# Kizuna42/office-person-detection-vit

Measured on AMD Instinct MI355X. Metric: frames/sec (Phase-2 DETR detect) at 800x1333 batch 8, higher is better.
Workload: dtype f16

## Files before the change

### office_person_detection_vit_amd/_capi.py

```python

from __future__ import annotations

import ctypes as C
import os
from typing import Optional

_HERE = os.path.dirname(os.path.abspath(__file__))
LIB_PATH = os.path.join(_HERE, "libopd_hip.so")
TEST_LIB_PATH = os.path.join(_HERE, "libopd_hip_test.so")

OPD_PIXELS_U8_BGR_HWC = 0
OPD_PIXELS_F32_NCHW = 1
OPD_MEM_HOST = 0
OPD_MEM_DEVICE = 1
OPD_MEM_HOST_PIXELS_DEVICE_OUT = 2
OPD_FLAG_NO_GRAPH = 1
OPD_FLAG_MULTI_STREAM = 2
OPD_REID_MODEL_CLIP = 0
OPD_REID_MODEL_OSNET = 1
OPD_FLAG_BF16 = 4
OPD_COMM_ID_BYTES = 128
OPD_OK, OPD_EINVAL, OPD_EIO, OPD_ESCHEMA, OPD_EHIP, OPD_ENOMEM, OPD_ESTATE = 0, -1, -2, -3, -4, -5, -6


# ... 39 lines not shown
    "opd_detr_forward_ragged": (C.c_int, [C.c_void_p, C.c_void_p, C.c_int, C.c_int, C.c_int, C.c_int, C.c_int, C.c_void_p,
                                          C.c_void_p, C.c_void_p, C.c_void_p]),
    "opd_detr_forward_resized": (C.c_int, [C.c_void_p, C.c_void_p] + [C.c_int] * 6 + [C.c_void_p] * 3),
    "opd_detr_resize_u8": (C.c_int, [C.c_void_p, C.c_void_p] + [C.c_int] * 5 + [C.c_void_p]),
    "opd_detr_detect_resized": (C.c_int, [C.c_void_p, C.c_void_p] + [C.c_int] * 6 + [C.c_float, C.POINTER(OpdDet), C.POINTER(C.c_int32)]),
    "opd_detr_detect_frames": (C.c_int, [C.c_void_p, C.POINTER(C.c_void_p)] + [C.c_int] * 6 + [C.c_float, C.POINTER(OpdDet), C.POINTER(C.c_int32)]),
    "opd_detr_detect_frames_features": (C.c_int, [C.c_void_p, C.POINTER(C.c_void_p)] + [C.c_int] * 5 + [C.c_float, C.c_int, C.POINTER(OpdDet), C.POINTER(C.c_int32),
                                                   C.POINTER(C.c_float)]),
    "opd_detr_postprocess": (C.c_int, [C.c_void_p, C.c_float, C.c_void_p, C.POINTER(OpdDet), C.POINTER(C.c_int32)]),
    "opd_detr_detect": (C.c_int, [C.c_void_p, C.c_void_p, C.c_int, C.c_int, C.c_int, C.c_int, C.c_int, C.c_float,
                                  C.c_void_p, C.POINTER(OpdDet), C.POINTER(C.c_int32)]),
    "opd_detr_detect_ragged": (C.c_int, [C.c_void_p, C.c_void_p, C.c_int, C.c_int, C.c_int, C.c_int, C.c_int, C.c_void_p,
                                         C.c_float, C.c_void_p, C.POINTER(OpdDet), C.POINTER(C.c_int32)]),
    "opd_detr_detect_async": (C.c_int, [C.c_void_p, C.c_void_p, C.c_int, C.c_int, C.c_int, C.c_int, C.c_int, C.c_float, C.c_void_p,
                                        C.POINTER(OpdDet), C.POINTER(C.c_int32), C.POINTER(C.c_int)]),
    "opd_detr_wait": (C.c_int, [C.c_void_p, C.c_int]),
    "opd_person_nms": (C.c_int, [C.POINTER(OpdDet), C.c_int, C.c_int, C.c_float]),
    "opd_person_nms_batch": (C.c_int, [C.POINTER(OpdDet), C.POINTER(C.c_int32), C.c_int, C.c_int, C.c_int, C.c_float]),
    "opd_host_alloc": (C.c_int, [C.c_size_t, C.POINTER(C.c_void_p)]),
    "opd_host_free": (None, [C.c_void_p]),
    "opd_similarity_matrix": (C.c_int, [C.c_int, C.c_void_p, C.c_void_p, C.c_void_p, C.c_int, C.c_void_p, C.c_void_p, C.c_void_p, C.c_int,
                                        C.c_int, C.c_double, C.c_double, C.c_int, C.c_void_p]),
    "opd_detr_roi_features": (C.c_int, [C.c_void_p, C.c_int, C.c_void_p, C.c_int, C.c_int, C.c_int, C.c_void_p]),
    "opd_detr_attention_map": (C.c_int, [C.c_void_p, C.c_int, C.c_int, C.c_void_p, C.c_int, C.c_void_p, C.c_int]),
    "opd_detr_set_profiling": (C.c_int, [C.c_void_p, C.c_int]),
    "opd_detr_stage_times": (C.c_int, [C.c_void_p, C.POINTER(C.c_float)]),
    "opd_detr_kernel_times": (C.c_int, [C.c_void_p, C.POINTER(C.c_float), C.POINTER(C.c_int32), C.POINTER(C.c_double)]),
    "opd_detr_kernel_table": (C.c_int, [C.c_void_p, C.c_void_p, C.c_int, C.POINTER(C.c_int)]),
    "opd_comm_available": (C.c_int, []),
    "opd_comm_unique_id": (C.c_int, [C.c_void_p]),
    "opd_comm_create": (C.c_int, [C.c_void_p, C.c_int, C.c_int, C.c_void_p, C.POINTER(C.c_void_p)]),
    "opd_comm_attach": (C.c_int, [C.c_void_p, C.c_void_p, C.POINTER(C.c_void_p)]),
    "opd_comm_destroy": (None, [C.c_void_p]),
    "opd_comm_info": (C.c_int, [C.c_void_p, C.POINTER(C.c_int), C.POINTER(C.c_int)]),
    "opd_comm_begin": (C.c_int, [C.c_void_p, C.c_int]),
    "opd_comm_detect": (C.c_int, [C.c_void_p, C.c_int, C.c_void_p, C.c_int, C.c_int, C.c_int, C.c_int, C.c_int, C.c_float, C.c_void_p]),
    "opd_comm_buffers": (C.c_int, [C.c_void_p, C.c_int, C.POINTER(C.c_void_p), C.POINTER(C.c_void_p)]),
    "opd_comm_exchange": (C.c_int, [C.c_void_p]),
    "opd_comm_wait": (C.c_int, [C.c_void_p, C.POINTER(OpdDet), C.POINTER(C.c_int32)]),
    "opd_reid_create": (C.c_int, [C.POINTER(OpdReidConfig), C.c_char_p, C.c_int, C.POINTER(C.c_void_p)]),
    "opd_reid_destroy": (None, [C.c_void_p]),
    "opd_reid_info": (C.c_int, [C.c_void_p, C.POINTER(OpdReidModelInfo)]),
    "opd_reid_extract": (C.c_int, [C.c_void_p, C.POINTER(C.c_void_p), C.c_void_p, C.c_int, C.c_int, C.c_void_p, C.c_void_p, C.c_int,
                                   C.c_void_p]),
    "opd_last_error": (C.c_char_p, []),
    "opd_version": (C.c_char_p, []),
}

TEST_API = {
    "opd_test_conv_gemm": (C.c_int, [C.c_void_p] * 6 + [C.c_int] * 15),
    "opd_test_gemm_splitk_ln": (C.c_int, [C.c_void_p] * 8 + [C.c_int] * 3),
    "opd_test_gemm_k256": (C.c_int, [C.c_void_p] * 5 + [C.c_int] * 5),
    "opd_test_gemm_ln": (C.c_int, [C.c_void_p] * 8 + [C.c_int] * 2),
    "opd_test_bench_gemm_ln": (C.c_int, [C.c_int] * 4 + [C.POINTER(C.c_float)]),
    "opd_test_gemm_ln_deep": (C.c_int, [C.c_void_p] * 7 + [C.c_int] + [C.c_void_p] * 3 + [C.c_int] * 3),
    "opd_test_set_heads2": (C.c_int, [C.c_int]),
    "opd_test_enc_ffn": (C.c_int, [C.c_void_p] * 9 + [C.c_int] + [C.c_void_p] * 3 + [C.c_int] * 3 + [C.c_void_p] * 2 + [C.c_int] * 2 + [C.c_void_p] * 5 + [C.c_int]),
    "opd_test_bench_enc_ffn": (C.c_int, [C.c_int] * 6 + [C.POINTER(C.c_float)]),
    "opd_test_bench_conv": (C.c_int, [C.c_int] * 11 + [C.POINTER(C.c_float)]),
    "opd_test_trace_btail": (C.c_int, [C.c_int] * 6 + [C.POINTER(C.c_ulonglong), C.c_int, C.POINTER(C.c_int)]),
    "opd_test_trace_conv": (C.c_int, [C.c_int] * 10 + [C.POINTER(C.c_ulonglong), C.c_int, C.POINTER(C.c_int)]),
    "opd_test_btail": (C.c_int, [C.c_void_p] * 10 + [C.c_int] * 6),
    "opd_test_bench_btail": (C.c_int, [C.c_int] * 8 + [C.POINTER(C.c_float)]),
    "opd_test_btail_repeat": (C.c_int, [C.c_void_p] * 8 + [C.c_int] * 6 + [C.POINTER(C.c_int)]),
    "opd_test_attention": (C.c_int, [C.c_void_p] * 4 + [C.c_int] * 4 + [C.c_float]),
    "opd_test_layernorm": (C.c_int, [C.c_void_p] * 5 + [C.c_int]),
    "opd_test_maxpool": (C.c_int, [C.c_void_p] * 2 + [C.c_int] * 6),
    "opd_test_preprocess_u8": (C.c_int, [C.c_void_p] * 2 + [C.c_int] * 5 + [C.c_void_p]),
    "opd_test_attention_masked": (C.c_int, [C.c_void_p] * 4 + [C.c_int] * 4 + [C.c_float, C.c_void_p, C.c_int]),
    "opd_test_stem2": (C.c_int, [C.c_void_p] * 4 + [C.c_int] * 5),
    "opd_test_stem_pool": (C.c_int, [C.c_void_p] * 4 + [C.c_int] * 7),
    "opd_test_set_fuse_stem_pool": (C.c_int, [C.c_void_p, C.c_int]),
    "opd_test_set_pos_shadow": (C.c_int, [C.c_void_p, C.c_int]),
    "opd_test_stem_pool_u8": (C.c_int, [C.c_void_p] * 6 + [C.c_int] * 3),
    "opd_test_set_fuse_btail": (C.c_int, [C.c_void_p, C.c_int]),
    "opd_test_set_fuse_gemm_ln": (C.c_int, [C.c_void_p, C.c_int]),
    "opd_test_f32_to_f16": (C.c_uint16, [C.c_float]),
    "opd_test_f16_to_f32": (C.c_float, [C.c_uint16]),
    "opd_test_normalise_key": (C.c_int, [C.c_char_p, C.c_char_p, C.c_int]),
    "opd_test_inspect_checkpoint": (C.c_int, [C.c_char_p, C.POINTER(C.c_int32)]),
    "opd_test_resize_coeffs": (C.c_int, [C.c_int, C.c_int, C.c_void_p, C.c_void_p, C.c_int]),
    "opd_test_valid_prefix": (C.c_int, [C.c_int] * 3),
    "opd_test_trunk_plan": (C.c_int, [C.c_void_p] + [C.c_int] * 6 + [C.c_void_p, C.c_int, C.c_void_p]),
    "opd_test_sine_pos_embed": (C.c_int, [C.c_int] * 5 + [C.c_void_p]),
    "opd_test_conv_dual": (C.c_int, [C.c_void_p] * 6 + [C.c_int] * 13),
    "opd_test_btail_sc": (C.c_int, [C.c_void_p] * 11 + [C.c_int] * 3),
    "opd_test_btail_chain": (C.c_int, [C.c_void_p] * 13 + [C.c_int] * 4),
    "opd_test_bench_attention": (C.c_int, [C.c_void_p] * 3 + [C.c_int] * 6 + [C.c_float, C.c_int, C.POINTER(C.c_float)]),
    "opd_test_trace_attention": (C.c_int, [C.c_void_p] * 3 + [C.c_int] * 6 + [C.c_float, C.c_void_p, C.c_int, C.POINTER(C.c_int)]),
    "opd_test_heads": (C.c_int, [C.c_void_p] * 13 + [C.c_int] * 2),
    "opd_test_postprocess": (C.c_int, [C.c_void_p] * 3 + [C.c_int] * 3 + [C.c_float, C.c_void_p, C.c_void_p]),
    "opd_test_roi_features": (C.c_int, [C.c_void_p] * 2 + [C.c_int] * 3 + [C.c_void_p]),
    "opd_test_set_conv_flags": (C.c_int, [C.c_int]),
    "opd_test_set_gemm_ln_kloop": (C.c_int, [C.c_int]),
    "opd_test_set_graph_guard": (C.c_int, [C.c_int]),
    "opd_test_set_alloc_poison": (C.c_int, [C.c_int]),
    "opd_test_check_redzones": (C.c_int, [C.c_void_p]),
    "opd_test_set_taps": (C.c_int, [C.c_void_p, C.c_int]),
    "opd_test_read_taps": (C.c_int, [C.c_void_p, C.c_void_p, C.c_int, C.c_char_p, C.c_int]),
    "opd_test_round_f16_diffused": (C.c_int, [C.c_void_p, C.c_int, C.c_int, C.c_int]),
    "opd_test_dec_qkv": (C.c_int, [C.c_void_p, C.c_void_p, C.c_int] + [C.c_void_p] * 5 + [C.c_int] * 2 + [C.c_void_p] * 4),
    "opd_test_dec_self": (C.c_int, [C.c_void_p] * 10 + [C.c_int, C.c_int, C.c_float, C.c_void_p]),
    "opd_test_attention_split": (C.c_int, [C.c_void_p] * 3 + [C.c_int] * 4 + [C.c_float, C.c_int, C.c_void_p, C.c_int, C.c_void_p, C.c_void_p]),
    "opd_test_dec_cross_out": (C.c_int, [C.c_void_p, C.c_void_p, C.c_int, C.c_void_p, C.c_int] + [C.c_void_p] * 4 + [C.c_int, C.c_void_p]),
    "opd_test_dec_ffn": (C.c_int, [C.c_void_p] * 4 + [C.c_int, C.c_int, C.c_void_p]),
    "opd_test_bench_dec": (C.c_int, [C.c_int] * 6 + [C.POINTER(C.c_float)]),
    "opd_test_heads_fused": (C.c_int, [C.c_void_p, C.c_void_p, C.c_int] + [C.c_void_p] * 13 + [C.c_int, C.c_int, C.c_void_p, C.c_void_p]),
    "opd_test_set_fused_dec": (C.c_int, [C.c_void_p, C.c_int]),
    "opd_test_set_elem_bf16": (C.c_int, [C.c_int]),
    "opd_test_trace_dec_self": (C.c_int, [C.c_int, C.c_int, C.c_void_p]),
    "opd_test_reid_geometry": (C.c_int, [C.c_void_p, C.c_int, C.c_int, C.c_int, C.c_void_p]),
    "opd_test_reid_coeffs": (C.c_int, [C.c_int] * 4 + [C.c_void_p, C.c_void_p, C.c_int]),
    "opd_test_reid_lut": (C.c_int, [C.c_void_p]),
    "opd_test_reid_pixels_host": (C.c_int, [C.c_void_p, C.c_int, C.c_int, C.c_void_p] + [C.c_int] * 3 + [C.c_void_p]),
    "opd_test_reid_pixels": (C.c_int, [C.c_void_p, C.POINTER(C.c_void_p), C.c_void_p, C.c_int, C.c_int, C.c_void_p, C.c_void_p, C.c_int,
                                       C.c_void_p]),
    "opd_test_reid_attention": (C.c_int, [C.c_void_p, C.c_void_p] + [C.c_int] * 3),
    "opd_test_reid_layernorm": (C.c_int, [C.c_void_p] * 5 + [C.c_int] * 3),
    "opd_test_reid_gemm": (C.c_int, [C.c_int, C.c_void_p, C.c_void_p, C.c_void_p, C.c_int, C.c_void_p] + [C.c_int] * 3),
    "opd_test_reid_l2norm": (C.c_int, [C.c_void_p] + [C.c_int] * 2),
    "opd_test_osnet_lut": (C.c_int, [C.c_void_p]),
    "opd_test_osnet_geometry": (C.c_int, [C.c_void_p, C.c_int, C.c_int, C.c_int, C.c_void_p]),
    "opd_test_osnet_pixels_host": (C.c_int, [C.c_void_p, C.c_int, C.c_int, C.c_void_p, C.c_int, C.c_void_p]),
    "opd_test_osnet_stem": (C.c_int, [C.c_void_p] * 4 + [C.c_int] * 2),
    "opd_test_osnet_gemm": (C.c_int, [C.c_int, C.c_void_p, C.c_int, C.c_int, C.c_void_p, C.c_int, C.c_int, C.c_void_p, C.c_void_p, C.c_void_p,
                                      C.c_int, C.c_void_p] + [C.c_int] * 6),
    "opd_test_osnet_dwconv": (C.c_int, [C.c_void_p] * 4 + [C.c_int] * 7),
    "opd_test_osnet_gate": (C.c_int, [C.c_void_p] * 7 + [C.c_int] * 4),
    "opd_test_osnet_avgpool2": (C.c_int, [C.c_void_p] * 2 + [C.c_int] * 4),
    "opd_test_osnet_head": (C.c_int, [C.c_void_p] * 4 + [C.c_int] * 3),
    "opd_test_reid_kernel_table": (C.c_int, [C.c_void_p, C.POINTER(C.c_void_p), C.c_void_p, C.c_int, C.c_void_p, C.c_void_p, C.c_int, C.c_int,
                                             C.POINTER(OpdKernelStat), C.c_int, C.POINTER(C.c_int)]),
}

_lib: Optional[C.CDLL] = None
_lib_has_hooks = False


def load_library(test_hooks: bool = False) -> C.CDLL:
    global _lib, _lib_has_hooks
    test_hooks = test_hooks or os.environ.get("OPD_TEST_HOOKS") == "1"
    if _lib is not None:
        if test_hooks and not _lib_has_hooks:
            raise RuntimeError("the product library is already loaded in this process; load the test build first "
                               "(_capi.load_library(test_hooks=True) or OPD_TEST_HOOKS=1)")
        return _lib
    path = TEST_LIB_PATH if test_hooks else LIB_PATH
    if not os.path.exists(path):
        raise RuntimeError(
            f"HIP extension not built: {path} is missing (run `python -c 'import __graft_entry__ as g; g.build()'`). "
            "This package has no CPU fallback.")
    lib = C.CDLL(path)
    for table in (API, TEST_API) if test_hooks else (API,):
        for name, (res, args) in table.items():
            fn = getattr(lib, name)
            fn.restype = res
            fn.argtypes = args
    _lib, _lib_has_hooks = lib, test_hooks
    return lib


def last_error() -> str:
    return load_library().opd_last_error().decode("utf-8", "replace")


def check(rc: int, what: str) -> None:
# ... 3 lines not shown
```

### office_person_detection_vit_amd/csrc/build.py

```python

from __future__ import annotations

import os
import subprocess
import sys

HERE = os.path.dirname(os.path.abspath(__file__))
PKG = os.path.dirname(HERE)
SOURCES = ["kernels_gemm.hip", "kernels_w8.hip", "kernels_btail.hip", "kernels_btail3.hip", "kernels_rowln.hip", "kernels_attn.hip", "kernels_misc.hip", "kernels_dec.hip", "kernels_reid.hip", "kernels_osnet.hip", "opd_loader.cpp", "opd_host.cpp", "opd_model.cpp", "opd_comm.cpp", "opd_dispatch.cpp", "opd_reid.cpp", "opd_osnet.cpp", "opd_test_api.cpp", "opd_reid_test_api.cpp", "opd_osnet_test_api.cpp"]
TEST_ONLY = {"opd_test_api.cpp", "opd_reid_test_api.cpp", "opd_osnet_test_api.cpp"}
ELEM_SOURCES = ["kernels_gemm.hip", "kernels_w8.hip", "kernels_btail.hip", "kernels_btail3.hip", "kernels_rowln.hip", "kernels_attn.hip", "kernels_misc.hip"]
HEADERS = ["opd_kernels.h", "opd_elem.h", "opd_loader.h", "opd_host.h", "opd_model.h", "opd_reid.h", "opd_osnet.h", os.path.join("..", "..", "include", "opd_detr.h")]
COMMON_FLAGS = ["-O3", "-fPIC", "-std=c++17", "--offload-arch=gfx950", "-Wall", "-Wno-unused-function", "-fvisibility=hidden"]
EXTRA_FLAGS = {"kernels_attn.hip": ["-mllvm", "-amdgpu-mfma-vgpr-form"]}
BF16_FLAGS = ["-DOPD_ELEM_BF16=1"]


def hipcc_path() -> str:
    return os.environ.get("HIPCC", "/opt/rocm/bin/hipcc")


LIB = os.path.join(PKG, "libopd_hip.so")
TEST_LIB = os.path.join(PKG, "libopd_hip_test.so")


def _stale(target: str, deps) -> bool:
    if not os.path.exists(target):
        return True
    t = os.path.getmtime(target)
    return any(os.path.getmtime(d) >= t for d in deps)


def build(verbose: bool = False, force: bool = False) -> str:
    hipcc = hipcc_path()
    objdir = os.path.join(HERE, "build")
    os.makedirs(objdir, exist_ok=True)
    hdrs = [os.path.join(HERE, h) for h in HEADERS]
    objs = []
    common, extra = COMMON_FLAGS, EXTRA_FLAGS
    jobs = []
    for src in SOURCES:
        sp = os.path.join(HERE, src)
        obj = os.path.join(objdir, os.path.splitext(src)[0] + ".o")
        objs.append(obj)
        if force or _stale(obj, [sp] + hdrs):
            jobs.append([hipcc] + common + extra.get(src, []) + (["-x", "hip"] if src.endswith(".cpp") else []) + ["-c", sp, "-o", obj])
        if src in ELEM_SOURCES:
            obj16 = os.path.join(objdir, os.path.splitext(src)[0] + "_bf16.o")
            objs.append(obj16)
            if force or _stale(obj16, [sp] + hdrs):
                jobs.append([hipcc] + common + extra.get(src, []) + BF16_FLAGS + ["-c", sp, "-o", obj16])

    def compile_one(cmd):
        if verbose:
            print(" ".join(cmd), flush=True)
        subprocess.run(cmd, check=True)

    if jobs:
        from concurrent.futures import ThreadPoolExecutor
        cores = int(os.environ.get("MAX_JOBS") or 0) or len(os.sched_getaffinity(0))
        with ThreadPoolExecutor(max_workers=max(1, min(len(jobs), cores))) as pool:
            list(pool.map(compile_one, jobs))
    test_objs = {os.path.join(objdir, os.path.splitext(s)[0] + ".o") for s in TEST_ONLY}
    for lib, members in ((LIB, [o for o in objs if o not in test_objs]), (TEST_LIB, objs)):
        if force or _stale(lib, members):
            cmd = [hipcc, "-shared", "-fPIC", "--offload-arch=gfx950", "-o", lib] + members + ["-ldl"]
            if verbose:
                print(" ".join(cmd), flush=True)
            subprocess.run(cmd, check=True)
    return LIB


if __name__ == "__main__":
    print(build(verbose=True, force="--force" in sys.argv))
```

### office_person_detection_vit_amd/csrc/kernels_btail.hip

```cpp
#include <hip/hip_runtime.h>
#include "opd_kernels.h"
#include "opd_elem.h"

typedef elem_t half8 __attribute__((ext_vector_type(8)));
typedef float float4v __attribute__((ext_vector_type(4)));
typedef unsigned int uint2v __attribute__((ext_vector_type(2)));
typedef unsigned int uint4v __attribute__((ext_vector_type(4)));

namespace {

constexpr int ROW_BYTES = 128;
constexpr int NW = 4;

__device__ __forceinline__ int swz(int row, int chunk) { return row * ROW_BYTES + ((chunk ^ (row & 7)) << 4); }

__device__ __forceinline__ int xcd_logical_block(int bid, int nblocks) {
    const int q = nblocks >> 3, r = nblocks & 7;
    const int x = bid & 7, k = bid >> 3;
    return (x < r ? x * (q + 1) : r * (q + 1) + (x - r) * q) + k;
}

__device__ __forceinline__ int own_row(const int rho) { return (rho & ~31) | (((rho >> 2) & 3) << 3) | (((rho >> 4) & 1) << 2) | (rho & 3); }
__device__ __forceinline__ int own_ch(const int nt, const int g) { return (nt >> 1) * 32 + g * 8 + (nt & 1) * 4; }

// ... 420 lines not shown
            }
        if constexpr (C3 > 0) {
            const unsigned char* W3s = W2s + W2C_BYTES;
#pragma unroll
            for (int kk = 0; kk < 2; ++kk) {
#pragma unroll
                for (int nt = 0; nt < NT3; ++nt) {
                    const half8 wf = *reinterpret_cast<const half8*>(W3s + swz(nt * 16 + li, kk * 4 + g));
#pragma unroll
                    for (int mt = 0; mt < 2; ++mt) accz[nt][mt] = OPD_MFMA_16x16x32(wf, yf[kk][mt], accz[nt][mt]);
                }
            }
        }
        if (j + 1 < NCH) {
            if (res_dma && j + 2 < NCH) wait_vmcnt<4>();
            else wait_vmcnt<0>();
            __builtin_amdgcn_s_barrier();
        }
#pragma unroll
        for (int q = 0; q < 2; ++q)
#pragma unroll
            for (int mt = 0; mt < 2; ++mt)
                if (y_ok[mt] && !(p.dbg & 2)) *reinterpret_cast<half8*>(p.y + pr_row[mt] + j * 64 + q * 32) = yf[q][mt];
        stamp(4 + j);
    }

    if constexpr (C3 > 0) {
#pragma unroll
        for (int q = 0; q < NT3 / 2; ++q)
#pragma unroll
            for (int mt = 0; mt < 2; ++mt) {
                float4v v0 = accz[2 * q][mt], v1 = accz[2 * q + 1][mt];
#pragma unroll
                for (int r = 0; r < 4; ++r) {
                    v0[r] = v0[r] > 0.f ? v0[r] : 0.f;
                    v1[r] = v1[r] > 0.f ? v1[r] : 0.f;
                }
                if (pr_ok[mt] && !(p.dbg & 2))
                    *reinterpret_cast<uint4*>(p.z + (size_t)(wm0 + mt * 16 + li) * C3 + q * 32 + g * 8) =
                        make_uint4(pack2h(v0[0], v0[1]), pack2h(v0[2], v0[3]), pack2h(v1[0], v1[1]), pack2h(v1[2], v1[3]));
            }
    }
    if constexpr (TRACE) {
        stamp(4 + NCH);
        asm volatile("s_waitcnt vmcnt(0)" ::: "memory");
        stamp(5 + NCH);
        asm volatile("s_memrealtime %0\n\ts_waitcnt lgkmcnt(0)" : "=s"(tstamp[15])::"memory");
        if (threadIdx.x == 0 && p.trace) {
#pragma unroll
            for (int i = 0; i < 16; ++i) p.trace[(size_t)blockIdx.x * 16 + i] = tstamp[i];
        }
    }
#endif
}

template <int C1, int C3, bool RDMA, bool SC = false, bool TRACE = false, int RC = 0>
hipError_t launch_btail_t(const BtailParams& p, hipStream_t stream) {
    constexpr int BM = 32 * NW;
    constexpr int MAIN = (BM + C1) * ROW_BYTES, CHUNK = 64 * C1 * 2 + C3 * ROW_BYTES + (SC ? 64 * ROW_BYTES : 0) + (RC ? 2 * 64 * ROW_BYTES : 0);
    constexpr int LDS = 2 * (MAIN > CHUNK ? MAIN : CHUNK) + (RDMA ? 2 * NW * 4096 : 0);
    static_assert(LDS <= 160 * 1024, "LDS per workgroup");
    OPD_SET_MAX_LDS_ONCE((btail_kernel<C1, C3, RDMA, SC, TRACE, RC>), LDS);
    OPD_LAUNCH((btail_kernel<C1, C3, RDMA, SC, TRACE, RC>), dim3((p.M + BM - 1) / BM), dim3(64 * NW), LDS, stream, p);
    static const char* const kname = opd_kernel_name("btail_kernel<%d, %d, %s, %s, %s, %d>", C1, C3, OPD_BOOLSTR(RDMA), OPD_BOOLSTR(SC), OPD_BOOLSTR(TRACE), RC);
    opd_last_kernel_name = kname;
    return hipGetLastError();
}

}

#ifndef OPD_ELEM_BF16
bool opd_btail_supported(int C1, int C3) {
    return (C1 == 64 && (C3 == 0 || C3 == 64 || C3 == 128)) || (C1 == 128 && (C3 == 0 || C3 == 128)) || opd_btail256_supported(C1, C3);
}
#endif

hipError_t OPD_SYM(opd_launch_btail)(const BtailParams& p_in, hipStream_t stream) {
    if (!opd_btail_supported(p_in.C1, p_in.C3) || p_in.OH <= 0 || p_in.OW <= 0) return hipErrorInvalidValue;
    BtailParams p = p_in;
    p.fd_ohw = opd_make_fastdiv((unsigned)p.OH * (unsigned)p.OW);
    p.fd_ow = opd_make_fastdiv((unsigned)p.OW);
    if ((size_t)p.B * p.H * p.W * p.C1 * 2 + (size_t)(p.W + 1) * p.C1 * 2 >= 0x7fffff00ull) return hipErrorInvalidValue;
    if ((size_t)p.M * p.C1 * 8 >= 0x7fffff00ull) return hipErrorInvalidValue;
    if (p.C1 == 256) return OPD_SYM(opd_launch_btail256)(p, stream);
    if (p.y_stride2 && (p.stride != 1 || p.C3 == 0)) return hipErrorInvalidValue;
    if (!p.y && !p.a1_out) return hipErrorInvalidValue;
    if (p.rc) {
        if (p.rc != 1 || p.C1 != 64 || p.C3 != 64 || p.stride != 1 || p.res || p.xs || !p.rc_a1 || !p.rc_xs || !p.rc_w2 || !p.rc_wsc || !p.rc_b ||
            p.trace || (size_t)p.M * 64 * 2 >= 0x7fffff00ull)
            return hipErrorInvalidValue;
        return launch_btail_t<64, 64, false, false, false, 1>(p, stream);
    }
    if (p.xs) {
        if (p.C1 != 64 || p.C3 != 64 || p.stride != 1 || !p.wsc || p.res || (size_t)p.M * 64 * 2 >= 0x7fffff00ull) return hipErrorInvalidValue;
        return launch_btail_t<64, 64, false, true>(p, stream);
    }
    if (p.trace) {
        if (p.C1 == 64 && p.C3 == 64 && (p.dbg & 16)) return launch_btail_t<64, 64, false, false, true>(p, stream);
        if (p.C1 == 64 && p.C3 == 64) return launch_btail_t<64, 64, true, false, true>(p, stream);
        if (p.C1 == 128 && p.C3 == 128) return launch_btail_t<128, 128, false, false, true>(p, stream);
        return hipErrorInvalidValue;
    }
    if (p.C1 == 64) {
        const bool rdma = !(p.dbg & 16);
        if (p.C3 == 0) return rdma ? launch_btail_t<64, 0, true>(p, stream) : launch_btail_t<64, 0, false>(p, stream);
        if (p.C3 == 64) return rdma ? launch_btail_t<64, 64, true>(p, stream) : launch_btail_t<64, 64, false>(p, stream);
        return rdma ? launch_btail_t<64, 128, true>(p, stream) : launch_btail_t<64, 128, false>(p, stream);
    }
    if (p.C3 == 0) return launch_btail_t<128, 0, false>(p, stream);
    return launch_btail_t<128, 128, false>(p, stream);
}

#ifndef OPD_ELEM_BF16
void opd_permute_k32(const f16_t* w, f16_t* out, int rows, int K) {
    for (int n = 0; n < rows; ++n)
        for (int b = 0; b < K; b += 32)
            for (int g = 0; g < 4; ++g)
                for (int e = 0; e < 4; ++e) {
                    out[(size_t)n * K + b + 8 * g + e] = w[(size_t)n * K + b + 4 * g + e];
                    out[(size_t)n * K + b + 8 * g + 4 + e] = w[(size_t)n * K + b + 16 + 4 * g + e];
                }
}
#endif
```

### office_person_detection_vit_amd/csrc/opd_kernels.h

```cpp
#pragma once
#include <hip/hip_runtime.h>
#include <stdint.h>
#include <vector>

typedef uint16_t f16_t;
enum { OPD_DT_F16 = 0, OPD_DT_BF16 = 1 };

#include <mutex>
#define OPD_SET_MAX_LDS_ONCE(kernel, bytes)                                                                                  \
    do {                                                                                                                     \
        static std::once_flag once_[16];                                                                                     \
        static hipError_t err_[16];                                                                                          \
        int dev_ = 0;                                                                                                        \
        if (hipGetDevice(&dev_) != hipSuccess || dev_ < 0 || dev_ >= 16) return hipErrorInvalidDevice;    \
        std::call_once(once_[dev_], [&] { err_[dev_] = hipFuncSetAttribute(reinterpret_cast<const void*>(kernel), hipFuncAttributeMaxDynamicSharedMemorySize, (bytes)); }); \
        if (err_[dev_] != hipSuccess) return err_[dev_];                                                                     \
    } while (0)

extern thread_local const char* opd_last_kernel_name;
extern thread_local int opd_dbg_skip_launch;
const char* opd_kernel_name(const char* fmt, ...);
#define OPD_LAUNCH(kernel, ...)                       \
    do {                                              \
        opd_last_kernel_name = #kernel;               \
// ... 7 lines not shown
        asm volatile("s_waitcnt vmcnt(0)" ::: "memory");         \
        __syncthreads();                                         \
    } while (0)
#else
#define OPD_DMA_BARRIER() __syncthreads()
#endif

struct FastDiv { unsigned mul, shift, one; };
inline FastDiv opd_make_fastdiv(unsigned d) {
    FastDiv f{0u, 0u, 1u};
    if (d <= 1u) return f;
    int s = 0;
    while ((1ull << s) < d) ++s;
    f.mul = (unsigned)(((1ull << (31 + s)) + d - 1) / d);
    f.shift = (unsigned)(s - 1);
    f.one = 0u;
    return f;
}

struct ConvGemmParams {
    const f16_t* x;
    const f16_t* w;
    const float* bias;
    const float* const* bias_ptrs;
    const f16_t* res16;
    const float* res32;
    void* out;
    f16_t* out16_aux;
    const void* zero16;
    int B, H, W, Cin, OH, OW, N, KH, KW, stride, pad;
    int M, K;
    int relu, bias_period, out_f32;
    int bias_pmod, bias_pcols;
    int stem;
    int dbg;
    int split_k;
    const f16_t* x2;
    int H2, W2, Cin2, stride2, K1;
    FastDiv fd_ohw, fd_ow, fd_period;
    const f16_t* x_alt;
    int alt_mod, alt_cols;
    unsigned tap_rep;
    FastDiv fd_tilesn, fd_ntiles;
    unsigned long long* trace;
    int force_mt;
    int wprefetch;
    int flat_staging;
    int dtype;
};
hipError_t opd_launch_conv_gemm(const ConvGemmParams& p, hipStream_t stream);
bool opd_conv_w8_supported(const ConvGemmParams& p);
hipError_t opd_launch_conv_w8(const ConvGemmParams& p, hipStream_t stream);
hipError_t opd_launch_stem_pool_u8(const uint8_t* frames, const int32_t* valid_hw, const f16_t* w, const float* bias, f16_t* out, int B, int H,
                                   int W, int OH, int OW, int PH, int PW, hipStream_t stream, int dtype = 0);
hipError_t opd_launch_stem_pool(const f16_t* x4p, const f16_t* w, const float* bias, f16_t* out, int B, int Hp, int Wp, int OH,
                                int OW, int PH, int PW, hipStream_t stream, int dtype = 0);
struct BtailParams {
    const f16_t* x1;
    const f16_t* w1;
    const float* b1;
    const f16_t* w2p;
    const float* b2;
    const f16_t* res;
    const f16_t* xs;
    const f16_t* wsc;
    f16_t* y;
    const f16_t* w3p;
    const float* b3;
    f16_t* z;
    int B, H, W, OH, OW, stride, M, C1, C3;
    int dbg;
    FastDiv fd_ohw, fd_ow;
    unsigned long long* trace;
    int rev;
    int dtype;
    f16_t* a1_out;
    const f16_t* rc_a1;
    const f16_t* rc_xs;
    const f16_t* rc_w2;
    const f16_t* rc_wsc;
    const float* rc_b;
    int rc;
    int y_stride2;
};
bool opd_btail_supported(int C1, int C3);
hipError_t opd_launch_btail(const BtailParams& p, hipStream_t stream);
void opd_permute_k32(const f16_t* w, f16_t* out, int rows, int K);
bool opd_btail256_supported(int C1, int C3);
hipError_t opd_launch_btail256(const BtailParams& p, hipStream_t stream);

struct GemmLnParams {
    const f16_t* x;
    const f16_t* w;
    const float* bias;
    const float* res32;
    const float* gamma;
    const float* beta;
    float* y32;
    f16_t* y16;
    int M, K;
    int kloop;
    int deep_k;
    const float* pos;
    const float* const* pos_ptrs;
    int pos_period;
    f16_t* yp16;
    int dtype;
};
hipError_t opd_launch_gemm_ln(const GemmLnParams& p, hipStream_t stream);
struct EncFfnParams {
    const f16_t* x;
    const unsigned char* wpack;
    const float* b2;
    const float* res32;
    const float* gamma;
    const float* beta;
    float* y32;
    f16_t* y16;
    f16_t* yp16;
    const float* pos;
    const float* const* pos_ptrs;
    int pos_period;
    int M, F;
    int dtype;
    int dbg;
    int wprefetch;
    const f16_t* attn;
    const float* bo;
    const float* gamma1;
    const float* beta1;
    int pack_front;
    int pack_tail;
    int tail, tail_pos;
    f16_t* tail_out;
    int tail_ld;
    int tail_col[16];
};
hipError_t opd_launch_enc_ffn(const EncFfnParams& p, hipStream_t stream);
size_t opd_encffn_pack_bytes(int F, int tail, int front);
void opd_encffn_pack(const uint16_t* w1, const float* b1, const uint16_t* w2, int F, const uint16_t* wt, const float* bt, int tail, const uint16_t* wo,
                     unsigned char* out);
struct GemmK256Params {
    const f16_t* x;
    const f16_t* w;
    const float* bias;
    f16_t* out16;
    float* out32;
    int M, N, ldx, ldw, slices, bias_period, relu;
    int dtype;
};
hipError_t opd_launch_gemm_k256(const GemmK256Params& p, hipStream_t stream);

hipError_t opd_launch_preprocess_u8(const uint8_t* frames, f16_t* out, int B, int H, int W, int Hp, int Wp, const int32_t* valid_hw,
                                    hipStream_t stream, int dtype = 0);
hipError_t opd_launch_preprocess_f32(const float* pv, f16_t* out, int B, int H, int W, int Hp, int Wp, const int32_t* valid_hw,
                                     hipStream_t stream, int dtype = 0);
void opd_resize_coeffs(int in_size, int out_size, std::vector<int32_t>* bounds, std::vector<int32_t>* coeffs, int* ksize_out);
hipError_t opd_launch_resize_u8(const uint8_t* in, uint8_t* out, int B, int h, int w, int oh, int ow, const int32_t* bounds_h,
                                const int32_t* coeff_h, int ksize_h, const int32_t* bounds_v, const int32_t* coeff_v, int ksize_v,
                                hipStream_t stream);
hipError_t opd_launch_maxpool(const f16_t* x, f16_t* out, int B, int H, int W, int C, int OH, int OW, hipStream_t stream, int dtype = 0);
hipError_t opd_launch_layernorm(const float* x, const float* gamma, const float* beta, float* y, f16_t* y16,
                                int rows, hipStream_t stream, int dtype = 0);
hipError_t opd_launch_reduce_ln(const float* partials, int nsplit, size_t slab_stride, const float* residual,
                                const float* gamma, const float* beta, float* y, f16_t* y16, int rows, hipStream_t stream, int dtype = 0);
hipError_t opd_launch_reduce_ln_pos(const float* partials, int nsplit, size_t slab_stride, const float* residual, const float* gamma,
                                    const float* beta, float* y, f16_t* y16, int rows, const float* pos, const float* const* pos_ptrs,
                                    int period, f16_t* yp16, hipStream_t stream, int dtype = 0);
hipError_t opd_launch_broadcast_rows(const float* c, float* y, f16_t* y16, int rows, hipStream_t stream, int dtype = 0);
hipError_t opd_launch_cast_f16(const float* x, f16_t* y, size_t n, hipStream_t stream, int dtype = 0);
hipError_t opd_launch_reduce_act16(const float* partials, int nsplit, size_t slab_stride, f16_t* out, size_t n, int relu, hipStream_t stream, int dtype = 0);
#define OPD_TAP_BLOCKS 64
// ... 35 lines not shown
hipError_t opd_launch_similarity_matrix(const float* f1, const float* b1, const uint8_t* has1, int n1, const float* f2, const float* b2,
                                        const uint8_t* has2, int n2, int D, double aw, double mw, int as_distance, float* out,
                                        hipStream_t stream);

void opd_split_f16_frag(const float* w, int N, int K, f16_t* out);
struct DecQkvParams {
    const float* h_in;
    const float* partials;
    int nsplit;
    const float* b2;
    const float *ln_g, *ln_b;
    float* h_out;
    const f16_t* w;
    const float* bias;
    f16_t* q16;
    f16_t* k16;
    f16_t* vT;
    int M, Q;
};
hipError_t opd_launch_dec_qkv(const DecQkvParams& p, hipStream_t stream);
struct DecSelfParams {
    const f16_t *q16, *k16, *vT;
    float* h;
    const f16_t* wo;
    const float *bo, *ln_g, *ln_b;
    const f16_t* wq;
    const float* rbq;
    f16_t* qc16;
    int qc_bf16;
    int B, Q;
    float scale;
    unsigned long long* trace;
};
hipError_t opd_launch_dec_self(const DecSelfParams& p, hipStream_t stream);
struct DecCrossOutParams {
    const float* part_o;
    const float* part_ml;
    int splits;
    const float* res;
    int res_period;
    float* h;
    const f16_t* wo;
    const float *bo, *ln_g, *ln_b;
    int M;
};
hipError_t opd_launch_dec_cross_out(const DecCrossOutParams& p, hipStream_t stream);
#define OPD_DEC_FFN_CHUNK 128
struct DecFfnParams {
    const float* h;
    const f16_t* w1;
    const float* b1;
    const f16_t* w2;
    float* partials;
    int M, F;
};
hipError_t opd_launch_dec_ffn(const DecFfnParams& p, hipStream_t stream);

struct AttnParams {
    const f16_t *q, *k, *v;
    f16_t* o;
    int B, heads, Lq, Lk;
    int ldq, ldk, ldv, ldo;
    float scale;
    const int32_t* key_valid;
    int key_row;
    unsigned long long* trace;
    int splits;
    float *part_o, *part_ml;
    int dtype;
};
hipError_t opd_launch_attention(const AttnParams& p, hipStream_t stream);

#define OPD_DECL_ELEM(name, ...)          \
    hipError_t name##_f16(__VA_ARGS__);   \
    hipError_t name##_bf16(__VA_ARGS__);
OPD_DECL_ELEM(opd_launch_conv_gemm, const ConvGemmParams& p, hipStream_t stream)
OPD_DECL_ELEM(opd_launch_conv_w8, const ConvGemmParams& p, hipStream_t stream)
OPD_DECL_ELEM(opd_launch_stem_pool_u8, const uint8_t* frames, const int32_t* valid_hw, const f16_t* w, const float* bias, f16_t* out, int B, int H, int W, int OH,
              int OW, int PH, int PW, hipStream_t stream)
OPD_DECL_ELEM(opd_launch_stem_pool, const f16_t* x4p, const f16_t* w, const float* bias, f16_t* out, int B, int Hp, int Wp, int OH, int OW, int PH, int PW,
              hipStream_t stream)
OPD_DECL_ELEM(opd_launch_btail, const BtailParams& p, hipStream_t stream)
OPD_DECL_ELEM(opd_launch_btail256, const BtailParams& p, hipStream_t stream)
OPD_DECL_ELEM(opd_launch_gemm_ln, const GemmLnParams& p, hipStream_t stream)
OPD_DECL_ELEM(opd_launch_enc_ffn, const EncFfnParams& p, hipStream_t stream)
OPD_DECL_ELEM(opd_launch_gemm_k256, const GemmK256Params& p, hipStream_t stream)
OPD_DECL_ELEM(opd_launch_attention, const AttnParams& p, hipStream_t stream)
OPD_DECL_ELEM(opd_launch_attention_map, const f16_t* q, int ldq, const f16_t* k, int ldk, const int32_t* sel, int nsel, int heads, int Lk, float scale,
              const int32_t* key_valid2, int key_row, void* stat, float* out, hipStream_t stream)
OPD_DECL_ELEM(opd_launch_preprocess_u8, const uint8_t* frames, f16_t* out, int B, int H, int W, int Hp, int Wp, const int32_t* valid_hw, hipStream_t stream)
OPD_DECL_ELEM(opd_launch_preprocess_f32, const float* pv, f16_t* out, int B, int H, int W, int Hp, int Wp, const int32_t* valid_hw, hipStream_t stream)
OPD_DECL_ELEM(opd_launch_maxpool, const f16_t* x, f16_t* out, int B, int H, int W, int C, int OH, int OW, hipStream_t stream)
OPD_DECL_ELEM(opd_launch_layernorm, const float* x, const float* gamma, const float* beta, float* y, f16_t* y16, int rows, hipStream_t stream)
OPD_DECL_ELEM(opd_launch_broadcast_rows, const float* c, float* y, f16_t* y16, int rows, hipStream_t stream)
OPD_DECL_ELEM(opd_launch_reduce_ln, const float* partials, int nsplit, size_t slab_stride, const float* residual, const float* gamma, const float* beta, float* y,
              f16_t* y16, int rows, hipStream_t stream)
OPD_DECL_ELEM(opd_launch_reduce_ln_pos, const float* partials, int nsplit, size_t slab_stride, const float* residual, const float* gamma, const float* beta,
              float* y, f16_t* y16, int rows, const float* pos, const float* const* pos_ptrs, int period, f16_t* yp16, hipStream_t stream)
OPD_DECL_ELEM(opd_launch_cast_f16, const float* x, f16_t* y, size_t n, hipStream_t stream)
OPD_DECL_ELEM(opd_launch_reduce_act16, const float* partials, int nsplit, size_t slab_stride, f16_t* out, size_t n, int relu, hipStream_t stream)
```

### office_person_detection_vit_amd/csrc/opd_model.cpp

```cpp
#include <new>
#include <stdexcept>

#include "opd_model.h"

using namespace opd;


namespace opd {

std::atomic<int> g_alloc_poison{-1};

static int upload_f32(opd_detr* m, float** dst, const std::vector<float>& v) {
    RCCHK(dalloc(m, dst, v.size(), true));
    HIPCHK(hipMemcpy(*dst, v.data(), v.size() * 4, hipMemcpyHostToDevice));
    return OPD_OK;
}
static int upload_f16(opd_detr* m, f16_t** dst, const std::vector<float>& v) {
    std::vector<f16_t> h(v.size());
    if (m->dtype == OPD_DT_BF16) for (size_t i = 0; i < v.size(); ++i) h[i] = f32_to_bf16(v[i]);
    else for (size_t i = 0; i < v.size(); ++i) h[i] = f32_to_f16(v[i]);
    RCCHK(dalloc(m, dst, h.size(), true));
    HIPCHK(hipMemcpy(*dst, h.data(), h.size() * 2, hipMemcpyHostToDevice));
    return OPD_OK;
}
// ... 587 lines not shown

static int run_small_gemm(opd_detr* m, const f16_t* x, const f16_t* w, const float* bias, int bias_period, int M, int N, int K,
                          f16_t* out16, bool relu) {
    GemmK256Params p{}; p.dtype = m->dtype;
    p.x = x; p.w = w; p.bias = bias; p.out16 = out16; p.M = M; p.N = N; p.ldx = K; p.ldw = K; p.slices = 1;
    p.bias_period = bias_period; p.relu = relu ? 1 : 0;
    RCCHK(timed_begin(m, CLS_GEMM, 2.0 * M * (double)N * K));
    HIPCHK(opd_launch_gemm_k256(p, m->stream));
    RCCHK(timed_end(m));
    RCCHK(tap(m, "gemm_k256", out16, (size_t)M * N * 2));
    return OPD_OK;
}
static int run_small_gemm_ln(opd_detr* m, const f16_t* x, const f16_t* w, const float* bias, int M, int K, const float* res32,
                             const LNp& ln, float* y32, f16_t* y16) {
    GemmK256Params p{}; p.dtype = m->dtype;
    p.x = x; p.w = w; p.bias = bias; p.out32 = m->d_slab; p.M = M; p.N = 256; p.ldx = K; p.ldw = K; p.slices = K / 256;
    RCCHK(timed_begin(m, CLS_GEMM, 2.0 * M * 256.0 * K));
    HIPCHK(opd_launch_gemm_k256(p, m->stream));
    RCCHK(timed_end(m));
    RCCHK(timed_begin(m, CLS_OTHER, 0.0));
    HIPCHK(opd_launch_reduce_ln(m->d_slab, p.slices, (size_t)M * 256, res32, ln.g, ln.b, y32, y16, M, m->stream, m->dtype));
    RCCHK(timed_end(m));
    RCCHK(tap(m, "small_gemm_ln", y32, (size_t)M * 256 * 4));
    return OPD_OK;
}

static int run_attn(opd_detr* m, const f16_t* q, int ldq, const f16_t* k, int ldk, const f16_t* v, int ldv, f16_t* o, int ldo,
                    int B, int Lq, int Lk, const int32_t* key_valid = nullptr, int key_row = 0) {
    AttnParams p{}; p.dtype = m->dtype;
    p.key_valid = key_valid; p.key_row = key_row;
    p.q = q; p.k = k; p.v = v; p.o = o; p.B = B; p.heads = m->arch.heads; p.Lq = Lq; p.Lk = Lk;
    p.ldq = ldq; p.ldk = ldk; p.ldv = ldv; p.ldo = ldo;
    p.scale = 1.0f / sqrtf((float)(m->arch.d_model / m->arch.heads));
    RCCHK(timed_begin(m, CLS_ATTN, 4.0 * B * (double)m->arch.heads * Lq * Lk * 32));
    HIPCHK(opd_launch_attention(p, m->stream));
    RCCHK(timed_end(m));
    if (ldo == m->arch.d_model) RCCHK(tap(m, "attention", o, (size_t)B * Lq * ldo * 2));
    return OPD_OK;
}

TrunkPlan plan_trunk(const Arch& a, const std::vector<Block>& blocks, const opd_config& cfg, const Switches& sw, int B, int H2, int W2, int num_cus,
                     bool taps, int profiling, bool has_stream2) {
    TrunkPlan plan;
    plan.steps.resize(blocks.size());
    plan.split = B;
    const bool multi = (cfg.flags & OPD_FLAG_MULTI_STREAM) != 0;
    int ch = H2, cw = W2, oh3 = 0, ow3 = 0;
    for (int s = 0, bi = 0; s < 4; ++s) {
        for (int l = 0; l < a.depths[s]; ++l, ++bi) {
            const Block& b = blocks[bi];
            const Block* nbk = bi + 1 < (int)blocks.size() ? &blocks[bi + 1] : nullptr;
            const int oh = (b.c1.stride == 2) ? down2(ch) : ch, ow = (b.c1.stride == 2) ? down2(cw) : cw;
            const int C1 = b.c1.Cin;
            const bool sc_in_tail = b.has_sc && sw.fuse_shortcut && sw.fuse_btail && block_has_bias2sc(b) && b.sc.KH == 1 && b.sc.stride == 1 &&
                                    b.sc.Cin == 64 && b.c1.Cin == 64 && b.c1.stride == 1 && b.c2.Cout == 256 && nbk && conv_has_kperm(nbk->c0) &&
                                    nbk->c0.Cin == 256 && nbk->c0.Cout == 64;
            bool tail = sw.fuse_btail && b.c1.KH == 3 && b.c1.Cout == C1 && b.c2.Cin == C1 && b.c2.Cout == 4 * C1 && conv_has_kperm(b.c2) &&
                        opd_btail_supported(C1, 0);
            if (sw.dual_over_tail && tail && b.has_sc && !sc_in_tail && block_has_w2sc(b)) tail = false;
            if (C1 == 256 && tail) {
                const long long tiles = ((long long)cfg.max_batch * oh * ow + 127) / 128;
                const bool pays = tiles * 10 >= (long long)num_cus * 6;
                if (sw.tail3 == 0 || (sw.tail3 == 1 && !pays && !multi)) tail = false;
            }
            const bool sc_in_expand = b.has_sc && sw.fuse_shortcut && block_has_w2sc(b) && !sc_in_tail && !tail;
            tail = tail && (size_t)B * ch * cw * C1 * 2 < 0x7ff00000ull;
            TrunkStep& t = plan.steps[bi];
            t.path = tail ? PATH_TAIL : sc_in_expand ? PATH_DUAL : PATH_CONVS;
            t.sc = !b.has_sc ? SC_NONE : (sc_in_tail && tail) ? SC_TAIL : sc_in_expand ? SC_EXPAND : SC_LAUNCH;
            t.res = (t.sc == SC_TAIL || t.sc == SC_EXPAND) ? RES_NONE : t.sc == SC_LAUNCH ? RES_SHORTCUT : RES_TRUNK;
            t.store = STORE_Y;
            t.C3 = 0;
            if (tail && nbk && conv_has_kperm(nbk->c0) && nbk->c0.Cin == 4 * C1 && opd_btail_supported(C1, nbk->c0.Cout)) t.C3 = nbk->c0.Cout;
            if (tail && sw.y_stride2 && t.C3 && b.c1.stride == 1 && l + 1 == a.depths[s] && nbk && nbk->has_sc && nbk->sc.stride == 2 && nbk->sc.KH == 1 &&
                nbk->c1.stride == 2 && !taps)
                t.store = STORE_Y_STRIDE2;
            if (l > 0 && sw.tail_rc && !taps) {
                TrunkStep& prev = plan.steps[bi - 1];
                if (prev.path == PATH_TAIL && prev.sc == SC_TAIL && prev.C3 == 64 && prev.store == STORE_Y && tail && C1 == 64 && t.C3 == 64 &&
                    t.res == RES_TRUNK) {
                    prev.store = STORE_A1;
                    t.res = RES_REBUILD;
                }
            }
            if (s == 2 && l == 0) { oh3 = oh; ow3 = ow; }
            ch = oh; cw = ow;
        }
    }
    const int s3 = a.depths[0] + a.depths[1], s4 = s3 + a.depths[2];
    bool fused3 = a.depths[2] > 2 && profiling != 1 && !taps && has_stream2 && sw.tail3_split && !multi && B >= 2;
    for (int bi = s3 + 1; bi < s4 && fused3; ++bi) fused3 = plan.steps[bi].path == PATH_TAIL;
    if (fused3) {
        auto tiles_of = [&](int frames) { return ((long long)frames * oh3 * ow3 + 127) / 128; };
        const long long total = tiles_of(B), cus = num_cus, last = total % cus;
        if (total > cus && last > 0 && last < cus / 2) {
            const long long whole = (total / cus) * cus;
            int bA = B - 1;
            while (bA > 1 && tiles_of(bA) > whole) --bA;
            if (tiles_of(bA) <= whole) plan.split = bA;
        }
    }
    int n = 0;
    auto rev = [&](const TrunkStep& t) { return t.path == PATH_TAIL && sw.tail_rev ? (n++ & 1) : 0; };
    for (int bi = 0; bi < s4; ++bi) plan.steps[bi].rev = rev(plan.steps[bi]);
    for (int bi = s3 + 1; bi < s4 && plan.split < B; ++bi) plan.steps[bi].rev_b = rev(plan.steps[bi]);
    for (int bi = s4; bi < (int)blocks.size(); ++bi) plan.steps[bi].rev = rev(plan.steps[bi]);
    return plan;
}

#define MARK(i)                                                   \
    do {                                                          \
        if (m->profiling) HIPCHK(hipEventRecord(m->ev[i], m->stream)); \
        opd_dbg_skip_launch = (m->sw.dbg_skip >> (i)) & 1;           \
    } while (0)

static bool is_ragged(const int32_t* valid_hw, int B, int H, int W) {
    if (!valid_hw) return false;
    for (int b = 0; b < B; ++b)
        if (valid_hw[2 * b] != H || valid_hw[2 * b + 1] != W) return true;
    return false;
}

static int enqueue_forward(opd_detr* m, const void* d_pixels, int pixel_format, int B, int H, int W, const int32_t* valid_hw = nullptr) {
    const Arch& a = m->arch;
    Dims d;
    compute_dims(B, H, W, &d);
    const int fh = d.sh[3], fw = d.sw[3];
    const bool ragged = is_ragged(valid_hw, B, H, W);
    Plan* plan = nullptr;
    const float* const* enc_bias_ptrs[16] = {};
    const float* const* kv_bias_ptrs = nullptr;
    const float* const* pos_ptrs = nullptr;
    const int32_t *d_valid = nullptr, *d_keyv = nullptr;
    if (!ragged) {
        RCCHK(get_plan(m, fh, fw, fh, fw, &plan));
    } else {
        if (a.enc_layers > 16) return fail(OPD_EINVAL, "ragged batches: at most 16 encoder layers");
        m->h_valid_hw.assign(valid_hw, valid_hw + 2 * B);
        m->h_key_valid.resize((size_t)2 * B);
        m->h_bias_ptrs.assign((size_t)(a.enc_layers + 2) * B, nullptr);
        for (int b = 0; b < B; ++b) {
            const int vh = valid_hw[2 * b], vw = valid_hw[2 * b + 1];
            if (vh < 1 || vw < 1 || vh > H || vw > W) return fail(OPD_EINVAL, "valid_hw outside the frame canvas");
            const int vfh = valid_prefix(vh, H, fh), vfw = valid_prefix(vw, W, fw);
            if (vfh < 1 || vfw < 1) return fail(OPD_EINVAL, "frame too small: no valid feature-map position");
            m->h_key_valid[2 * b] = vfh; m->h_key_valid[2 * b + 1] = vfw;
            Plan* pb = nullptr;
            RCCHK(get_plan(m, fh, fw, vfh, vfw, &pb));
            if (b == 0) plan = pb;
            for (int i = 0; i < a.enc_layers; ++i) m->h_bias_ptrs[(size_t)i * B + b] = pb->rb_enc[i];
            m->h_bias_ptrs[(size_t)a.enc_layers * B + b] = pb->rb_kv;
            m->h_bias_ptrs[(size_t)(a.enc_layers + 1) * B + b] = pb->d_pos;
        }
        HIPCHK(hipMemcpyAsync(m->d_valid_hw, m->h_valid_hw.data(), (size_t)2 * B * 4, hipMemcpyHostToDevice, m->stream));
        HIPCHK(hipMemcpyAsync(m->d_key_valid, m->h_key_valid.data(), (size_t)2 * B * 4, hipMemcpyHostToDevice, m->stream));
        HIPCHK(hipMemcpyAsync(m->d_bias_ptrs, m->h_bias_ptrs.data(), m->h_bias_ptrs.size() * sizeof(float*), hipMemcpyHostToDevice, m->stream));
        for (int i = 0; i < a.enc_layers; ++i) enc_bias_ptrs[i] = m->d_bias_ptrs + (size_t)i * B;
        kv_bias_ptrs = m->d_bias_ptrs + (size_t)a.enc_layers * B;
        pos_ptrs = m->d_bias_ptrs + (size_t)(a.enc_layers + 1) * B;
        d_valid = m->d_valid_hw;
        d_keyv = m->d_key_valid;
    }
    timed_reset(m);
    m->tap_next = 0;
    if (pixel_format == OPD_PIXELS_U8_BGR_HWC) RCCHK(tap(m, "pixels_u8", d_pixels, (size_t)B * H * W * 3));
    MARK(0);
    const int Hp = 2 * d.H1 + 6, Wp = 2 * d.W1 + 6;
    const bool prep_in_stem = m->sw.fuse_prep && m->sw.fuse_stem_pool && pixel_format == OPD_PIXELS_U8_BGR_HWC;
    if (!prep_in_stem) {
        RCCHK(timed_begin(m, CLS_OTHER, 0.0));
        if (pixel_format == OPD_PIXELS_U8_BGR_HWC)
            HIPCHK(opd_launch_preprocess_u8(reinterpret_cast<const uint8_t*>(d_pixels), m->d_x4, B, H, W, Hp, Wp, d_valid, m->stream, m->dtype));
        else
            HIPCHK(opd_launch_preprocess_f32(reinterpret_cast<const float*>(d_pixels), m->d_x4, B, H, W, Hp, Wp, d_valid, m->stream, m->dtype));
        RCCHK(timed_end(m));
    }
    if (prep_in_stem) {
        RCCHK(timed_begin(m, CLS_CONV, 2.0 * B * d.H1 * d.W1 * 64.0 * 147.0));
        HIPCHK(opd_launch_stem_pool_u8(reinterpret_cast<const uint8_t*>(d_pixels), d_valid, m->stem.w, m->stem.bias, m->d_pool, B, H, W, d.H1, d.W1,
                                       d.H2, d.W2, m->stream, m->dtype));
        RCCHK(timed_end(m));
        RCCHK(tap(m, "stem_pool_u8", m->d_pool, (size_t)B * d.H2 * d.W2 * 64 * 2));
    } else if (m->sw.fuse_stem_pool) {
        RCCHK(timed_begin(m, CLS_CONV, 2.0 * B * d.H1 * d.W1 * 64.0 * 147.0));
        HIPCHK(opd_launch_stem_pool(m->d_x4, m->stem.w, m->stem.bias, m->d_pool, B, Hp, Wp, d.H1, d.W1, d.H2, d.W2, m->stream, m->dtype));
        RCCHK(timed_end(m));
    } else {
        ConvGemmParams p{}; p.dtype = m->dtype;
        p.x = m->d_x4; p.w = m->stem.w; p.bias = m->stem.bias; p.out = m->d_stem; p.zero16 = m->zero_bias;
        p.B = B; p.H = Hp; p.W = Wp; p.Cin = 256; p.OH = d.H1; p.OW = d.W1; p.N = 64; p.KH = 1; p.KW = 1; p.stride = 2; p.pad = 0;
        p.M = B * d.H1 * d.W1; p.K = 256; p.relu = 1; p.stem = 2;
        RCCHK(timed_begin(m, CLS_CONV, 2.0 * p.M * 64.0 * 147.0));
        HIPCHK(opd_launch_conv_gemm(p, m->stream));
        RCCHK(timed_end(m));
        RCCHK(timed_begin(m, CLS_OTHER, 0.0));
        HIPCHK(opd_launch_maxpool(m->d_stem, m->d_pool, B, d.H1, d.W1, 64, d.H2, d.W2, m->stream, m->dtype));
        RCCHK(timed_end(m));
    }
    MARK(1);
    const TrunkPlan tp = plan_trunk(a, m->blocks, m->cfg, m->sw, B, d.H2, d.W2, m->num_cus, m->taps != 0, m->profiling, m->stream2 != nullptr);
    struct TrunkState { int cur_id; int ch, cw; int z_id; int prev_id; };
    auto run_blocks = [&](int s_begin, int s_end, int b0, int nb, TrunkState& st, int l_begin = 0, int l_end = 1 << 30) -> int {
        auto trunk = [&](int id, size_t per_frame) { return (id == 0 ? m->d_pool : id == 1 ? m->d_t0 : m->d_t1) + (size_t)b0 * per_frame; };
        auto mid = [&](int id, size_t per_frame) { return (id ? m->d_m1 : m->d_m0) + (size_t)b0 * per_frame; };
        for (int s = s_begin; s < s_end; ++s) {
            for (int l = l_begin; l < a.depths[s] && l < l_end; ++l) {
                const int bi = m->stage_first[s] + l;
                const Block& b = m->blocks[bi];
                const TrunkStep& t = tp.steps[bi];
                const int ch = st.ch, cw = st.cw;
                const int oh = (b.c1.stride == 2) ? down2(ch) : ch, ow = (b.c1.stride == 2) ? down2(cw) : cw;
                const int C1 = b.c1.Cin, C2 = b.c2.Cout, C3 = t.C3;
                const f16_t* cur = trunk(st.cur_id, (size_t)ch * cw * b.c0.Cin);
                const int out_id = st.cur_id == 1 ? 2 : 1;
                f16_t* out = trunk(out_id, (size_t)oh * ow * C2);
                f16_t* const scb = m->d_sc + (size_t)b0 * oh * ow * C2;
                if (t.sc == SC_LAUNCH) RCCHK(run_conv(m, b.sc, cur, nb, ch, cw, oh, ow, scb, false, nullptr));
                const f16_t* res = t.res == RES_TRUNK ? cur : t.res == RES_SHORTCUT ? scb : nullptr;
                int x1_id = st.z_id;
                const f16_t* x1 = nullptr;
                if (x1_id >= 0) {
                    x1 = mid(x1_id, (size_t)ch * cw * C1);
                } else {
                    x1_id = 0;
                    f16_t* c0out = mid(0, (size_t)ch * cw * b.c0.Cout);
                    RCCHK(run_conv(m, b.c0, cur, nb, ch, cw, ch, cw, c0out, true, nullptr, (l == 0 && s > 0) ? s - 1 : s));
                    x1 = c0out;
                }
                st.z_id = -1;
                if (t.path == PATH_TAIL) {
                    const Block* nbk = C3 ? &m->blocks[bi + 1] : nullptr;
                    BtailParams p{}; p.dtype = m->dtype;
                    p.x1 = x1; p.w1 = b.c1.w; p.b1 = b.c1.bias; p.w2p = C1 == 256 ? b.c2.wp : b.c2.w; p.b2 = b.c2.bias; p.res = res;
                    p.y = t.store == STORE_A1 ? nullptr : out;
                    if (t.sc == SC_TAIL) { p.xs = cur; p.wsc = b.sc.w; p.b2 = b.bias2sc; }
                    f16_t* z = mid(1 - x1_id, (size_t)oh * ow * C3);
                    if (C3) { p.w3p = C1 == 256 ? nbk->c0.wp : nbk->c0.w; p.b3 = nbk->c0.bias; p.z = z; }
                    f16_t* const a1_keep = m->d_sc + (size_t)b0 * oh * ow * C1;
                    if (t.store == STORE_A1) p.a1_out = a1_keep;
                    if (t.res == RES_REBUILD) {
                        const Block& pb = m->blocks[bi - 1];
                        p.rc = 1; p.rc_a1 = a1_keep; p.rc_xs = trunk(st.prev_id, (size_t)ch * cw * pb.c0.Cin); p.rc_w2 = pb.c2.w; p.rc_wsc = pb.sc.w; p.rc_b = pb.bias2sc;
                    }
                    p.y_stride2 = t.store == STORE_Y_STRIDE2;
                    p.B = nb; p.H = ch; p.W = cw; p.OH = oh; p.OW = ow; p.stride = b.c1.stride; p.M = nb * oh * ow; p.C1 = C1; p.C3 = C3;
                    p.rev = b0 ? t.rev_b : t.rev;
                    p.dbg = m->sw.dbg_btail;
                    RCCHK(timed_begin(m, CLS_CONV, 2.0 * p.M * ((double)C1 * 9 * C1 + 4.0 * C1 * C1 + 4.0 * C1 * C3 + (t.sc == SC_TAIL ? 64.0 * 256 : 0.0))));
                    HIPCHK(opd_launch_btail(p, m->stream));
                    RCCHK(timed_end(m));
                    if (p.y) RCCHK(tap(m, "btail_y", out, (size_t)p.M * 4 * C1 * 2));
                    if (C3) RCCHK(tap(m, "btail_z", z, (size_t)p.M * C3 * 2));
                    if (C3) st.z_id = 1 - x1_id;
                } else {
                    f16_t* a1 = mid(1 - x1_id, (size_t)oh * ow * C1);
                    RCCHK(run_conv(m, b.c1, x1, nb, ch, cw, oh, ow, a1, true, nullptr, s));
                    if (t.path == PATH_DUAL) {
                        ConvGemmParams p{}; p.dtype = m->dtype;
                        p.x = a1; p.w = b.w2sc; p.bias = b.bias2sc; p.out = out; p.zero16 = m->zero_bias;
                        p.B = nb; p.H = oh; p.W = ow; p.Cin = C1; p.OH = oh; p.OW = ow; p.N = C2; p.KH = 1; p.KW = 1; p.stride = 1; p.pad = 0;
                        p.M = nb * oh * ow; p.K1 = C1; p.K = C1 + b.sc.Cin; p.relu = 1;
                        p.x2 = cur; p.H2 = ch; p.W2 = cw; p.Cin2 = b.sc.Cin; p.stride2 = b.sc.stride; p.dbg = m->sw.dbg_gemm; p.wprefetch = m->sw.wprefetch & 1;
                        RCCHK(timed_begin(m, CLS_CONV, 2.0 * p.M * (double)C2 * p.K));
                        HIPCHK(opd_launch_conv_gemm(p, m->stream));
                        RCCHK(timed_end(m));
                        RCCHK(tap(m, "dual_expand", out, (size_t)p.M * C2 * 2));
                    } else {
                        RCCHK(run_conv(m, b.c2, a1, nb, oh, ow, oh, ow, out, true, res));
                    }
                }
                st.prev_id = st.cur_id; st.cur_id = out_id; st.ch = oh; st.cw = ow;
            }
            if (b0 + nb == B && l_end >= a.depths[s]) MARK(2 + s);
        }
        return OPD_OK;
    };
    TrunkState st{0, d.H2, d.W2, -1, -1};
    RCCHK(run_blocks(0, 2, 0, B, st));
    const int nbA = tp.split;
    RCCHK(run_blocks(2, 3, 0, B, st, 0, 1));
    if (nbA < B) {
        TrunkState ta = st, tb = st;
        HIPCHK(hipEventRecord(m->ev_fork, m->stream));
        HIPCHK(hipStreamWaitEvent(m->stream2, m->ev_fork, 0));
        hipStream_t main_stream = m->stream;
        const int rc_a = run_blocks(2, 3, 0, nbA, ta, 1);
        m->stream = m->stream2;
        const int rc_b = rc_a == OPD_OK ? run_blocks(2, 3, nbA, B - nbA, tb, 1) : OPD_OK;
        m->stream = main_stream;
        const hipError_t ej = hipEventRecord(m->ev_join, m->stream2);
        const hipError_t ew = ej == hipSuccess ? hipStreamWaitEvent(m->stream, m->ev_join, 0) : ej;
        RCCHK(rc_a);
        RCCHK(rc_b);
        HIPCHK(ew);
        MARK(4);
        st = ta;
    } else {
        RCCHK(run_blocks(2, 3, 0, B, st, 1));
    }
    RCCHK(run_blocks(3, 4, 0, B, st));
    const f16_t* cur = st.cur_id == 1 ? m->d_t0 : m->d_t1;
    const int ch = st.ch, cw = st.cw;
    const int hw = ch * cw, M = B * hw, D = a.d_model, F = a.ffn;
    const bool shadow = m->sw.pos_shadow && D == 256 && m->enc[0].bqkv && m->bkv_all;
    const PosShadow psh{plan->d_pos, pos_ptrs, hw, m->d_xp16};
    const PosShadow* ps = shadow ? &psh : nullptr;
    auto run_deep = [&](const f16_t* x, const Lin* lin, const f16_t* w, const float* bias, int K, const float* res32, const LNp* ln, int cls) -> int {
        GemmLnParams gp{}; gp.dtype = m->dtype;
        gp.x = x; gp.w = w; gp.bias = bias; gp.res32 = res32; gp.gamma = ln ? ln->g : nullptr; gp.beta = ln ? ln->b : nullptr;
        gp.y32 = m->d_x32; gp.y16 = m->d_x16; gp.M = M; gp.K = K; gp.deep_k = 1;
        if (ps) { gp.pos = ps->pos; gp.pos_ptrs = ps->pos_ptrs; gp.pos_period = ps->period; gp.yp16 = ps->yp16; }
        RCCHK(timed_begin(m, cls, 2.0 * M * (double)D * K));
        HIPCHK(opd_launch_gemm_ln(gp, m->stream));
        RCCHK(timed_end(m));
        RCCHK(tap(m, ln ? "fc2_ln_ring" : "input_proj_ring", m->d_x32, (size_t)M * D * 4));
        (void)lin;
        return OPD_OK;
    };
    const bool small_enc = m->sw.small_enc && (size_t)m->cfg.max_batch * m->stage_px[3] <= 1400;
    const int enc_splits = small_enc ? 8 : 4;
    const bool deep_ok = m->sw.deep_fc2 && D == 256 && !small_enc;
    if (deep_ok && m->proj.K % 64 == 0 && (size_t)M * m->proj.K * 2 < 0x7fffff00ull)
        RCCHK(run_deep(cur, nullptr, m->proj.w, m->proj.bias, m->proj.K, nullptr, nullptr, CLS_CONV));
    else
        RCCHK(run_gemm_splitk_ln(m, cur, m->proj.w, m->proj.bias, M, D, m->proj.K, (m->proj.K / 64) % enc_splits == 0 ? enc_splits : 4, nullptr, nullptr, m->d_x32, m->d_x16, CLS_CONV, ps));
    bool qkv_done = false, kv_done = false;
    const int Q = a.queries, Md = B * Q, NKV = a.dec_layers * 2 * D;
    for (int i = 0; i < a.enc_layers; ++i) {
        const EncLayer& L = m->enc[i];
        if (qkv_done) {
// ... 332 lines not shown
    }
    if (hw != m->h_orig_hw) {
        HIPCHK(hipStreamSynchronize(m->stream));
        m->h_orig_hw = hw;
        HIPCHK(hipMemcpyAsync(m->d_orig_hw, m->h_orig_hw.data(), m->h_orig_hw.size() * 4, hipMemcpyHostToDevice, m->stream));
    }
    PostParams pp{};
    pp.logits = m->d_logits; pp.boxes = m->d_boxes; pp.orig_hw = m->d_orig_hw;
    pp.records = dev_out ? dev_out : m->d_records;
    pp.counts = dev_counts ? dev_counts : m->d_counts;
    pp.B = B; pp.Q = m->arch.queries; pp.ncls = m->arch.ncls; pp.threshold = threshold;
    RCCHK(timed_begin(m, CLS_OTHER, 0.0));
    HIPCHK(opd_launch_postprocess(pp, m->stream));
    RCCHK(timed_end(m));
    MARK(8);
    return OPD_OK;
}

static int fetch_records(opd_detr* m, opd_det* out, int32_t* counts, int mem_kind, float* features = nullptr) {
    const int B = m->last_B, Q = m->arch.queries;
    if (!outputs_on_device(mem_kind)) {
        const size_t rec_bytes = (size_t)m->cfg.max_batch * Q * sizeof(opd_det);
        const size_t feat_off = reinterpret_cast<const char*>(m->d_feat_all) - reinterpret_cast<const char*>(m->d_records);
        const size_t feat_row = (size_t)Q * m->arch.d_model * 4;
        if (!m->sync_pinned) HIPCHK(hipHostMalloc(&m->sync_pinned, feat_off + (size_t)m->cfg.max_batch * feat_row, hipHostMallocDefault));
        HIPCHK(hipMemcpyAsync(m->sync_pinned, m->d_records, features ? feat_off + (size_t)B * feat_row : rec_bytes + (size_t)B * 4, hipMemcpyDeviceToHost, m->stream));
        HIPCHK(hipStreamSynchronize(m->stream));
        memcpy(out, m->sync_pinned, (size_t)B * Q * sizeof(opd_det));
        memcpy(counts, static_cast<char*>(m->sync_pinned) + rec_bytes, (size_t)B * 4);
        if (features) memcpy(features, static_cast<char*>(m->sync_pinned) + feat_off, (size_t)B * feat_row);
    }
    HIPCHK(hipStreamSynchronize(m->stream));
    if (m->profiling) {
        for (int i = 0; i < 8; ++i) {
            float ms = 0.f;
            hipEvent_t from = (i == 7 && m->profiling == 2 && m->graph_marks) ? m->ev[9] : m->ev[i];
            if (hipEventElapsedTime(&ms, from, m->ev[i + 1]) == hipSuccess) m->stage_ms[i] = ms;
            else (void)hipGetLastError();
        }
        if (m->profiling == 1) timed_collect(m);
    }
    return OPD_OK;
}

}

static hipError_t make_branch_stream(opd_detr* m) {
    hipError_t e = hipStreamCreateWithFlags(&m->stream2, hipStreamNonBlocking);
    if (e == hipSuccess) e = hipEventCreateWithFlags(&m->ev_fork, hipEventDisableTiming);
    if (e == hipSuccess) e = hipEventCreateWithFlags(&m->ev_join, hipEventDisableTiming);
    return e;
}
static void drop_streams(opd_detr* m) {
    if (m->ev_fork) (void)hipEventDestroy(m->ev_fork);
    if (m->ev_join) (void)hipEventDestroy(m->ev_join);
    if (m->stream2) (void)hipStreamDestroy(m->stream2);
    if (m->stream) (void)hipStreamDestroy(m->stream);
    m->ev_fork = m->ev_join = nullptr; m->stream2 = m->stream = nullptr;
}

static int create_impl(const opd_config* cfg, const char* weights_path, int device_ordinal, opd_detr** out);
static int clone_impl(const opd_detr* src, opd_detr** out);
template <typename F>
static int guarded(const char* what, F&& body) {
    try {
        return body();
    } catch (const std::bad_alloc&) {
        return fail(OPD_ENOMEM, std::string(what) + ": out of host memory");
    } catch (const std::out_of_range& e) {
        return fail(OPD_ESCHEMA, std::string(what) + ": weight file lacks a tensor the model needs (" + e.what() + ")");
    } catch (const std::exception& e) {
        return fail(OPD_EINVAL, std::string(what) + ": " + e.what());
    } catch (...) {
        return fail(OPD_EINVAL, std::string(what) + ": unknown C++ exception");
    }
}
static Switches read_switches(int flags) {
    Switches sw;
    auto env = [](const char* name, int* v) { if (const char* e = getenv(name)) *v = atoi(e); };
    env("OPD_DUAL_OVER_TAIL", &sw.dual_over_tail);
    env("OPD_TAIL_REV", &sw.tail_rev);
    env("OPD_TAIL3", &sw.tail3);
    env("OPD_TAIL_RC", &sw.tail_rc);
    sw.tail_rc = sw.tail_rc != 0;
    env("OPD_WPREFETCH", &sw.wprefetch);
    env("OPD_W8", &sw.w8);
    if (sw.w8 < 0) sw.w8 = (flags & OPD_FLAG_MULTI_STREAM) ? 1 : 0;
    env("OPD_SMALL_SPLITK", &sw.small_splitk);
    env("OPD_SMALL_ENC", &sw.small_enc);
    env("OPD_Y_STRIDE2", &sw.y_stride2);
    env("OPD_TAIL3_SPLIT", &sw.tail3_split);
    env("OPD_FUSE_PREP", &sw.fuse_prep);
    env("OPD_POS_SHADOW", &sw.pos_shadow);
    env("OPD_DEEP_FC2", &sw.deep_fc2);
    env("OPD_WROUND", &sw.wround);
    env("OPD_FUSED_DEC", &sw.fused_dec);
    env("OPD_FUSED_ENC_FFN", &sw.fused_enc_ffn);
    env("OPD_ENC_TAIL", &sw.enc_tail);
    env("OPD_ENC_FRONT", &sw.enc_front);
    env("OPD_HEADS2", &sw.heads2);
    env("OPD_DBG_DEC_LAYERS", &sw.dbg_dec_layers);
    env("OPD_DBG_BTAIL", &sw.dbg_btail);
    env("OPD_DBG_SKIP", &sw.dbg_skip);
    env("OPD_DBG_GEMM", &sw.dbg_gemm);
    return sw;
}

extern "C" {

const char* opd_version(void) { return "opd_hip 0.2 gfx950 (fp16 MFMA operands, fp32 accumulate; OPD_FLAG_BF16: bf16 operands)"; }

int opd_detr_create(const opd_config* cfg, const char* weights_path, int device_ordinal, opd_detr** out) {
    ApiScope api_scope;
    if (out) *out = nullptr;
    return guarded("opd_detr_create", [&] { return create_impl(cfg, weights_path, device_ordinal, out); });
}
int opd_detr_clone(const opd_detr* src, opd_detr** out) {
    ApiScope api_scope;
    if (out) *out = nullptr;
    return guarded("opd_detr_clone", [&] { return clone_impl(src, out); });
}
static int create_impl(const opd_config* cfg, const char* weights_path, int device_ordinal, opd_detr** out) {
    if (!cfg || !weights_path || !out) return fail(OPD_EINVAL, "opd_detr_create: null argument");
    if (cfg->struct_size != (int32_t)sizeof(opd_config)) return fail(OPD_EINVAL, "opd_config.struct_size mismatch");
    if (cfg->max_batch < 1 || cfg->max_height < 32 || cfg->max_width < 32) return fail(OPD_EINVAL, "opd_config maxima must be >= 1 x 32 x 32");
    *out = nullptr;
    StateDict sd;
    std::string err;
    int rc = load_safetensors(weights_path, &sd, &err);
    if (rc) return fail(rc, err);
    std::unique_ptr<opd_detr> m(new opd_detr());
    rc = infer_arch(sd, &m->arch, &err);
    if (rc) return fail(rc, err);
    m->cfg = *cfg;
    m->dtype = (cfg->flags & OPD_FLAG_BF16) ? OPD_DT_BF16 : OPD_DT_F16;
    m->sw = read_switches(cfg->flags);
    m->device = device_ordinal;
    int ndev = 0;
    if (hipGetDeviceCount(&ndev) != hipSuccess || ndev == 0)
        return fail(OPD_EHIP, "no HIP device visible (this library has no CPU fallback)");
    if (device_ordinal < 0 || device_ordinal >= ndev) return fail(OPD_EINVAL, "device_ordinal out of range");
    auto cleanup = [&](int code) {
        for (void* p : m->allocs) (void)hipFree(p);
        drop_streams(m.get());
        return code;
    };
    {
        hipError_t e = hipSetDevice(device_ordinal);
        if (e == hipSuccess) e = hipStreamCreateWithFlags(&m->stream, hipStreamNonBlocking);
        if (e == hipSuccess) e = make_branch_stream(m.get());
        if (e != hipSuccess) { drop_streams(m.get()); return fail(OPD_EHIP, std::string("device/stream setup failed: ") + hipGetErrorString(e)); }
        int cus = 0;
        if (hipDeviceGetAttribute(&cus, hipDeviceAttributeMultiprocessorCount, device_ordinal) == hipSuccess && cus > 0) m->num_cus = cus;
    }
    m->weights = std::make_shared<WeightSet>();
    m->weights->device = device_ordinal;
    if ((rc = build_weights(m.get(), sd))) return cleanup(rc);
    m->weights_sealed = true;
    if ((rc = build_workspace(m.get()))) return cleanup(rc);
    for (auto& e : m->ev)
        if (hipEventCreate(&e) != hipSuccess) return cleanup(fail(OPD_EHIP, "hipEventCreate failed"));
    *out = m.release();
    ++g_handle_epoch;
    return OPD_OK;
}

// ... 409 lines not shown
```

### office_person_detection_vit_amd/csrc/opd_model.h

```cpp
#pragma once
#include <math.h>
#include <stdlib.h>
#include <string.h>

#include <atomic>
#include <memory>
#include <mutex>
#include <shared_mutex>
#include <string>
#include <vector>

#include "../../include/opd_detr.h"
#include "opd_kernels.h"
#include "opd_loader.h"
#include "opd_host.h"

#define HIPCHK(expr)                                                                                           \
    do {                                                                                                       \
        hipError_t _e = (expr);                                                                                \
        if (_e != hipSuccess)                                                                                  \
            return opd::fail(OPD_EHIP, std::string(#expr) + " failed: " + hipGetErrorString(_e) + " (" + __FILE__ + \
                                           ":" + std::to_string(__LINE__) + ")");                              \
    } while (0)

// ... 7 lines not shown



struct Conv {
    f16_t* w = nullptr;
    f16_t* wp = nullptr;
    float* bias = nullptr;
    int Cin = 0, Cout = 0, KH = 1, KW = 1, stride = 1, pad = 0, K = 0;
    bool stem = false;
};
struct Lin {
    f16_t* w = nullptr;
    float* b = nullptr;
    int N = 0, K = 0;
};
struct LNp {
    float* g = nullptr;
    float* b = nullptr;
};
struct Block {
    Conv c0, c1, c2, sc;
    bool has_sc = false;
    float* bias2sc = nullptr;
    f16_t* w2sc = nullptr;
};
inline bool conv_has_kperm(const Conv& c) { return c.KH == 1 && c.KW == 1 && c.Cin % 32 == 0 && c.Cin <= 1024; }
inline bool block_has_bias2sc(const Block& b) { return b.has_sc && b.sc.Cout == b.c2.Cout; }
inline bool block_has_w2sc(const Block& b) {
    return block_has_bias2sc(b) && b.sc.KH == 1 && b.c2.KH == 1 && b.c2.Cout % 128 == 0 && b.c2.Cin >= 128;
}
struct EncLayer {
    f16_t* wqkv = nullptr;
    float* bqkv = nullptr;
    Lin o, fc1, fc2;
    LNp ln1, ln2;
    unsigned char* ffn_pack = nullptr;
    int tail = 0, tail_pos = 0, tail_ld = 0;
    int front = 0;
    int tail_col[16] = {};
};
struct DecLayer {
    f16_t* wqkv = nullptr;
    f16_t* wq_c = nullptr;
    Lin so, co, fc1, fc2;
    LNp ln1, ln2, ln3;
    float* rb_self = nullptr;
    float* rb_q = nullptr;
    f16_t *wqkv_f = nullptr, *so_f = nullptr, *wqc_f = nullptr, *co_f = nullptr, *fc1_f = nullptr, *fc2_f = nullptr;
};

struct Plan {
    int fh = 0, fw = 0;
    int vh = 0, vw = 0;
    std::vector<float*> rb_enc;
    float* rb_kv = nullptr;
    float* d_pos = nullptr;
};

struct Dims {
    int B, H, W, H1, W1, H2, W2;
    int sh[4], sw[4];
};

inline int down2(int n) { return (n - 1) / 2 + 1; }

struct Switches {
    int small_m_gemm = 1;
    int fuse_gemm_ln = 1;
    int deep_fc2 = 1;
    int fuse_dec0 = 1;
    int enc_front = 1;
    int enc_tail = 0;
    int fused_enc_ffn = 1;
    int fused_dec = 1;
    int dec_splits = 3;
    int heads2 = 1;
    int fuse_btail = 1;
    int fuse_shortcut = 1;
    int dual_over_tail = 1;
    int tail_rev = 1;
    int tail3 = 1;
    int tail3_split = 1;
    int tail_rc = 1;
    int y_stride2 = 1;
    int wprefetch = 3;
    int w8 = -1;
    int small_splitk = 1;
    int small_enc = 1;
    int fuse_stem_pool = 1;
    int fuse_prep = 1;
    int pos_shadow = 1;
    int wround = 1;
    int dbg_btail = 0, dbg_gemm = 0;
    int dbg_dec_layers = 1 << 20;
    int dbg_skip = 0;
};

enum TrunkPath { PATH_TAIL, PATH_CONVS, PATH_DUAL };
enum TrunkShortcut { SC_NONE, SC_TAIL, SC_EXPAND, SC_LAUNCH };
enum TrunkResidual { RES_NONE, RES_TRUNK, RES_SHORTCUT, RES_REBUILD };
enum TrunkStore { STORE_Y, STORE_A1, STORE_Y_STRIDE2 };
struct TrunkStep {
    int path, sc, res, store;
    int C3;
    int rev, rev_b;
};
struct TrunkPlan {
    std::vector<TrunkStep> steps;
    int split = 0;
};
TrunkPlan plan_trunk(const Arch& a, const std::vector<Block>& blocks, const opd_config& cfg, const Switches& sw, int B, int H2, int W2, int num_cus,
                     bool taps, int profiling, bool has_stream2);

}

using namespace opd;

struct RedZoned { void* base; size_t bytes; int poison; };
struct WeightSet {
    std::vector<void*> allocs;
    std::vector<RedZoned> zoned;
    int device = 0;
    std::mutex plan_mu;
    std::vector<std::unique_ptr<Plan>> plans;
    ~WeightSet() {
        (void)hipSetDevice(device);
        for (void* p : allocs) (void)hipFree(p);
    }
};

struct opd_detr {
    Arch arch;
    opd_config cfg{};
    Switches sw;
    int dtype = 0;
    int device = 0;
    hipStream_t stream = nullptr;
    hipStream_t stream2 = nullptr;
    hipEvent_t ev_fork = nullptr, ev_join = nullptr;
    std::vector<void*> allocs;
    std::vector<RedZoned> zoned;
    std::shared_ptr<WeightSet> weights;
    bool weights_sealed = false;
    int64_t weight_bytes = 0, workspace_bytes = 0;

    Conv stem;
    std::vector<Block> blocks;
    std::vector<int> stage_first;
    Conv proj;
    std::vector<EncLayer> enc;
    std::vector<DecLayer> dec;
    f16_t* wkv_all = nullptr;
    float* bkv_all = nullptr;
    float* dec0_h = nullptr;
    f16_t* qc0 = nullptr;
    LNp dec_ln;
    float *wc = nullptr, *bc = nullptr, *w1 = nullptr, *b1 = nullptr, *w2 = nullptr, *b2 = nullptr, *w3 = nullptr, *b3 = nullptr;
    f16_t *wc_f = nullptr, *w1_f = nullptr, *w2_f = nullptr;
    float* zero_bias = nullptr;

    std::vector<std::vector<float>> h_enc_cat_w, h_enc_cat_b;
    std::vector<float> h_kv_cat_w, h_kv_cat_b;

    uint8_t* d_u8 = nullptr;
    float* d_pv = nullptr;
    f16_t *d_x4 = nullptr, *d_stem = nullptr, *d_pool = nullptr, *d_t0 = nullptr, *d_t1 = nullptr, *d_m0 = nullptr,
          *d_m1 = nullptr, *d_sc = nullptr;
    float *d_x32 = nullptr, *d_y32 = nullptr, *d_slab = nullptr;
    f16_t* d_xp16 = nullptr;
    f16_t *d_x16 = nullptr, *d_qkv16 = nullptr, *d_attn16 = nullptr, *d_ffn16 = nullptr, *d_memkv16 = nullptr;
    float *d_h32 = nullptr, *d_yd32 = nullptr, *d_hs32 = nullptr;
    f16_t *d_h16 = nullptr, *d_qkvd16 = nullptr, *d_qd16 = nullptr, *d_attnd16 = nullptr, *d_ffnd16 = nullptr;
    f16_t *d_dq16 = nullptr, *d_dk16 = nullptr, *d_dvT = nullptr;
    float *d_part_o = nullptr, *d_part_ml = nullptr, *d_ffn_part = nullptr;
    float *d_logits = nullptr, *d_boxes = nullptr;
    opd_det* d_records = nullptr;
    int32_t *d_counts = nullptr, *d_orig_hw = nullptr;
    int32_t *d_valid_hw = nullptr, *d_key_valid = nullptr;
    const float** d_bias_ptrs = nullptr;
    std::vector<int32_t> h_valid_hw, h_key_valid;
    std::vector<const float*> h_bias_ptrs;
    hipEvent_t ev_async[4] = {};
    unsigned async_next = 0;
    bool async_pending[4] = {};
    struct AsyncHost { void* pinned = nullptr; opd_det* out = nullptr; int32_t* counts = nullptr; int B = 0; };
    AsyncHost async_host[4];
    void* sync_pinned = nullptr;
    float* d_feat_all = nullptr;
// ... 98 lines not shown
```

### office_person_detection_vit_amd/csrc/opd_test_api.cpp

```cpp
#include <string.h>

#include <string>
#include <cstring>
#include <vector>

#include "opd_model.h"

namespace {
int tfail(int code, const std::string& msg) {
    opd::g_err = msg;
    return code;
}
struct DevMem {
    std::vector<void*> ptrs;
    ~DevMem() {
        for (void* p : ptrs) (void)hipFree(p);
    }
    template <typename T>
    T* up(const T* host, size_t count) {
        void* d = nullptr;
        if (hipMalloc(&d, count * sizeof(T) + 16) != hipSuccess) return nullptr;
        ptrs.push_back(d);
        if (host && hipMemcpy(d, host, count * sizeof(T), hipMemcpyHostToDevice) != hipSuccess) return nullptr;
        return reinterpret_cast<T*>(d);
    }
};
#define TCHK(expr)                                                                                          \
    do {                                                                                                    \
        hipError_t _e = (expr);                                                                             \
        if (_e != hipSuccess) return tfail(OPD_EHIP, std::string(#expr) + ": " + hipGetErrorString(_e));    \
    } while (0)
}

#pragma GCC visibility push(default)
extern "C" {

static int g_conv_flags = 0, g_gemm_ln_kloop = 0, g_test_dtype = 0;
int opd_test_set_elem_bf16(int on) { g_test_dtype = on ? OPD_DT_BF16 : OPD_DT_F16; return OPD_OK; }
int opd_test_set_conv_flags(int flags) { g_conv_flags = flags; return OPD_OK; }
int opd_test_set_gemm_ln_kloop(int on) { g_gemm_ln_kloop = on ? 1 : 0; return OPD_OK; }
static void apply_conv_flags(ConvGemmParams& p, int flags) {
    p.force_mt = (flags >> 8) & 7;
    p.flat_staging = (flags >> 5) & 1;
}

int opd_test_conv_gemm(const uint16_t* x, const uint16_t* w, const float* bias, const uint16_t* res16, const float* res32,
                       void* out, int B, int H, int W, int Cin, int OH, int OW, int N, int KH, int KW, int stride, int pad,
                       int relu, int bias_period, int out_f32, int stem) {
    DevMem dm;
    const size_t M = (size_t)B * OH * OW;
    const int K = stem ? 256 : KH * KW * Cin;
    const size_t xin = (size_t)B * H * W * (stem ? 4 : Cin);
    ConvGemmParams p{}; p.dtype = g_test_dtype;
    p.x = dm.up(x, xin);
    p.w = dm.up(w, (size_t)N * K);
    p.bias = dm.up(bias, (size_t)N * (bias_period > 0 ? bias_period : 1));
    p.res16 = res16 ? dm.up(res16, M * N) : nullptr;
    p.res32 = res32 ? dm.up(res32, M * N) : nullptr;
    const size_t obytes = M * N * (out_f32 ? 4 : 2);
    p.out = dm.up<unsigned char>(nullptr, obytes);
    {
        const uint32_t zeros[8] = {0, 0, 0, 0, 0, 0, 0, 0};
        p.zero16 = dm.up(zeros, 8);
    }
    if (!p.zero16 || !p.x || !p.w || !p.bias || !p.out || (res16 && !p.res16) || (res32 && !p.res32)) return tfail(OPD_ENOMEM, "test alloc failed");
    p.B = B; p.H = H; p.W = W; p.Cin = Cin; p.OH = OH; p.OW = OW; p.N = N; p.KH = KH; p.KW = KW; p.stride = stride; p.pad = pad;
    p.M = (int)M; p.K = K; p.relu = relu; p.bias_period = bias_period; p.out_f32 = out_f32; p.stem = stem;
    apply_conv_flags(p, g_conv_flags);
    if (g_conv_flags & (1 << 12)) {
        if (!opd_conv_w8_supported(p)) return tfail(OPD_EINVAL, "conv_w8: shape outside the kernel's contract");
        TCHK(opd_launch_conv_w8(p, nullptr));
    } else {
        TCHK(opd_launch_conv_gemm(p, nullptr));
    }
    TCHK(hipDeviceSynchronize());
    TCHK(hipMemcpy(out, p.out, obytes, hipMemcpyDeviceToHost));
    return OPD_OK;
}

int opd_test_conv_dual(const uint16_t* x, const uint16_t* w1, const uint16_t* x2, const uint16_t* w2, const float* bias, uint16_t* out,
                       int B, int H, int W, int Cin, int KH, int stride, int pad, int N, int H2, int W2, int Cin2, int stride2, int relu) {
    DevMem dm;
    const int OH = (H + 2 * pad - KH) / stride + 1, OW = (W + 2 * pad - KH) / stride + 1;
    const size_t M = (size_t)B * OH * OW;
    const int K1 = KH * KH * Cin, K = K1 + Cin2;
    std::vector<uint16_t> wc((size_t)N * K);
    for (int n = 0; n < N; ++n) {
        memcpy(&wc[(size_t)n * K], w1 + (size_t)n * K1, (size_t)K1 * 2);
        memcpy(&wc[(size_t)n * K + K1], w2 + (size_t)n * Cin2, (size_t)Cin2 * 2);
    }
    ConvGemmParams p{}; p.dtype = g_test_dtype;
    p.x = dm.up(x, (size_t)B * H * W * Cin);
    p.x2 = dm.up(x2, (size_t)B * H2 * W2 * Cin2);
    p.w = dm.up(wc.data(), wc.size());
    p.bias = dm.up(bias, (size_t)N);
    p.out = dm.up<unsigned char>(nullptr, M * N * 2);
    const uint32_t zeros[8] = {0, 0, 0, 0, 0, 0, 0, 0};
    p.zero16 = dm.up(zeros, 8);
    if (!p.x || !p.x2 || !p.w || !p.bias || !p.out || !p.zero16) return tfail(OPD_ENOMEM, "test alloc failed");
    p.B = B; p.H = H; p.W = W; p.Cin = Cin; p.OH = OH; p.OW = OW; p.N = N; p.KH = KH; p.KW = KH; p.stride = stride; p.pad = pad;
    p.M = (int)M; p.K = K; p.K1 = K1; p.relu = relu; p.H2 = H2; p.W2 = W2; p.Cin2 = Cin2; p.stride2 = stride2;
    TCHK(opd_launch_conv_gemm(p, nullptr));
    TCHK(hipDeviceSynchronize());
    TCHK(hipMemcpy(out, p.out, M * N * 2, hipMemcpyDeviceToHost));
    return OPD_OK;
}

int opd_test_gemm_splitk_ln(const uint16_t* x, const uint16_t* w, const float* bias, const float* res32, const float* gamma,
                            const float* beta, float* y, uint16_t* y16, int M, int K, int splits) {
    DevMem dm;
    const int N = 256;
    ConvGemmParams p{}; p.dtype = g_test_dtype;
    p.x = dm.up(x, (size_t)M * K);
    p.w = dm.up(w, (size_t)N * K);
    p.bias = dm.up(bias, N);
    std::vector<float> zeros(N, 0.f);
    p.zero16 = dm.up(zeros.data(), N);
    float* slab = dm.up<float>(nullptr, (size_t)splits * M * N);
    const float* dres = res32 ? dm.up(res32, (size_t)M * N) : nullptr;
    const float* dg = gamma ? dm.up(gamma, N) : nullptr;
    const float* db = beta ? dm.up(beta, N) : nullptr;
// ... 218 lines not shown
    for (int i = 0; i < 2; ++i) TCHK(opd_launch_conv_gemm(p, nullptr));
    TCHK(hipEventRecord(a, nullptr));
    for (int i = 0; i < iters; ++i) TCHK(opd_launch_conv_gemm(p, nullptr));
    TCHK(hipEventRecord(b, nullptr));
    TCHK(hipEventSynchronize(b));
    float ms = 0.f;
    TCHK(hipEventElapsedTime(&ms, a, b));
    (void)hipEventDestroy(a); (void)hipEventDestroy(b);
    *us_out = ms * 1000.f / iters;
    return OPD_OK;
}

int opd_test_trace_conv(int B, int H, int W, int Cin, int N, int KH, int stride, int with_res, int split_k, int warm, unsigned long long* trace_out,
                        int max_wgs, int* wgs_out) {
    const int dbg = 0;
    DevMem dm;
    const int pad = KH / 2, OH = (H + 2 * pad - KH) / stride + 1, OW = (W + 2 * pad - KH) / stride + 1;
    const size_t M = (size_t)B * OH * OW, K = (size_t)KH * KH * Cin;
    ConvGemmParams p{}; p.dtype = g_test_dtype;
    uint16_t* x = dm.up<uint16_t>(nullptr, (size_t)B * H * W * Cin);
    uint16_t* w = dm.up<uint16_t>(nullptr, (size_t)N * K);
    float* bias = dm.up<float>(nullptr, N);
    uint16_t* res = with_res ? dm.up<uint16_t>(nullptr, M * N) : nullptr;
    uint16_t* out = dm.up<uint16_t>(nullptr, M * N * (split_k > 1 ? 2 * (size_t)split_k : 1));
    float* zero = dm.up<float>(nullptr, 4096);
    unsigned long long* tr = dm.up<unsigned long long>(nullptr, (size_t)max_wgs * 8);
    if (!x || !w || !bias || !out || !zero || !tr || (with_res && !res)) return tfail(OPD_ENOMEM, "trace alloc failed");
    TCHK(hipMemset(x, 0x2c, (size_t)B * H * W * Cin * 2));
    TCHK(hipMemset(w, 0x1c, (size_t)N * K * 2));
    TCHK(hipMemset(bias, 0, (size_t)N * 4));
    TCHK(hipMemset(zero, 0, 4096 * 4));
    TCHK(hipMemset(tr, 0, (size_t)max_wgs * 64));
    if (res) TCHK(hipMemset(res, 0x2c, M * N * 2));
    p.x = x; p.w = w; p.bias = bias; p.res16 = res; p.out = out; p.zero16 = zero;
    p.B = B; p.H = H; p.W = W; p.Cin = Cin; p.OH = OH; p.OW = OW; p.N = N; p.KH = KH; p.KW = KH; p.stride = stride; p.pad = pad;
    p.M = (int)M; p.K = (int)K; p.relu = 1; p.dbg = dbg;
    if (split_k > 1) { p.split_k = split_k; p.out_f32 = 1; p.relu = 0; }
    unsigned long long* tr3 = dm.up<unsigned long long>(nullptr, (size_t)3 * max_wgs * 8);
    if (!tr3) return tfail(OPD_ENOMEM, "trace alloc failed");
    TCHK(hipMemset(tr3, 0, (size_t)3 * max_wgs * 64));
    p.trace = tr;
    for (int i = 0; i < warm; ++i) TCHK(opd_launch_conv_gemm(p, nullptr));
    for (int i = 0; i < 3; ++i) {
        p.trace = tr3 + (size_t)i * max_wgs * 8;
        TCHK(opd_launch_conv_gemm(p, nullptr));
    }
    TCHK(hipDeviceSynchronize());
    TCHK(hipMemcpy(trace_out, tr3, (size_t)3 * max_wgs * 64, hipMemcpyDeviceToHost));
    const int bn = (N % 128 == 0) ? 128 : 64;
    (void)bn;
    *wgs_out = max_wgs;
    return OPD_OK;
}

int opd_test_btail(const uint16_t* x1, const uint16_t* w1, const float* b1, const uint16_t* w2, const float* b2,
                   const uint16_t* res, const uint16_t* w3, const float* b3, uint16_t* y, uint16_t* z, int B, int H, int W,
                   int C1, int C3, int stride) {
    if (!opd_btail_supported(C1, C3)) return tfail(OPD_EINVAL, "btail: unsupported (C1, C3)");
    DevMem dm;
    const int C2 = 4 * C1, OH = (H - 1) / stride + 1, OW = (W - 1) / stride + 1;
    const size_t M = (size_t)B * OH * OW;
    std::vector<uint16_t> w2p((size_t)C2 * C1), w3p((size_t)(C3 ? C3 : 1) * C2);
    if (C1 == 256) {
        opd_permute_k32(w2, w2p.data(), C2, C1);
        if (C3) opd_permute_k32(w3, w3p.data(), C3, C2);
    } else {
        w2p.assign(w2, w2 + (size_t)C2 * C1);
        if (C3) w3p.assign(w3, w3 + (size_t)C3 * C2);
    }
    BtailParams p{}; p.dtype = g_test_dtype;
    p.x1 = dm.up(x1, (size_t)B * H * W * C1);
    p.w1 = dm.up(w1, (size_t)C1 * 9 * C1);
    p.b1 = dm.up(b1, C1);
    p.w2p = dm.up(w2p.data(), w2p.size());
    p.b2 = dm.up(b2, C2);
    p.res = res ? dm.up(res, M * C2) : nullptr;
    p.y = dm.up<uint16_t>(nullptr, M * C2);
    p.w3p = C3 ? dm.up(w3p.data(), w3p.size()) : nullptr;
    p.b3 = C3 ? dm.up(b3, C3) : nullptr;
    p.z = C3 ? dm.up<uint16_t>(nullptr, M * C3) : nullptr;
    if (!p.x1 || !p.w1 || !p.b1 || !p.w2p || !p.b2 || !p.y || (res && !p.res) || (C3 && (!p.w3p || !p.b3 || !p.z)))
        return tfail(OPD_ENOMEM, "test alloc failed");
    p.B = B; p.H = H; p.W = W; p.OH = OH; p.OW = OW; p.stride = stride; p.M = (int)M; p.C1 = C1; p.C3 = C3;
    TCHK(opd_launch_btail(p, nullptr));
    TCHK(hipDeviceSynchronize());
    TCHK(hipMemcpy(y, p.y, M * C2 * 2, hipMemcpyDeviceToHost));
    if (C3) TCHK(hipMemcpy(z, p.z, M * C3 * 2, hipMemcpyDeviceToHost));
    return OPD_OK;
}

int opd_test_btail_repeat(const uint16_t* x1, const uint16_t* w1, const float* b1, const uint16_t* w2, const float* b2, const uint16_t* res,
                          const uint16_t* w3, const float* b3, int B, int H, int W, int C1, int C3, int reps, int* n_diff) {
    if (!opd_btail_supported(C1, C3) || !C3 || reps < 2 || !n_diff) return tfail(OPD_EINVAL, "btail_repeat: bad arguments");
    DevMem dm;
    const int C2 = 4 * C1;
    const size_t M = (size_t)B * H * W;
    std::vector<uint16_t> w2p((size_t)C2 * C1), w3p((size_t)C3 * C2);
    if (C1 == 256) {
        opd_permute_k32(w2, w2p.data(), C2, C1);
        opd_permute_k32(w3, w3p.data(), C3, C2);
    } else {
        w2p.assign(w2, w2 + (size_t)C2 * C1);
        w3p.assign(w3, w3 + (size_t)C3 * C2);
    }
    BtailParams p{}; p.dtype = g_test_dtype;
    p.x1 = dm.up(x1, M * C1); p.w1 = dm.up(w1, (size_t)C1 * 9 * C1); p.b1 = dm.up(b1, C1); p.w2p = dm.up(w2p.data(), w2p.size());
    p.b2 = dm.up(b2, C2); p.res = dm.up(res, M * C2); p.y = dm.up<uint16_t>(nullptr, M * C2); p.w3p = dm.up(w3p.data(), w3p.size());
    p.b3 = dm.up(b3, C3); p.z = dm.up<uint16_t>(nullptr, M * C3);
    const size_t noise_bytes = (size_t)256 << 20;
    unsigned char* noise = dm.up<unsigned char>(nullptr, 2 * noise_bytes);
    unsigned long long* sums = dm.up<unsigned long long>(nullptr, (size_t)reps * 2 * OPD_TAP_BLOCKS);
    if (!p.x1 || !p.w1 || !p.b1 || !p.w2p || !p.b2 || !p.res || !p.y || !p.w3p || !p.b3 || !p.z || !noise || !sums) return tfail(OPD_ENOMEM, "test alloc failed");
    p.B = B; p.H = H; p.W = W; p.OH = H; p.OW = W; p.stride = 1; p.M = (int)M; p.C1 = C1; p.C3 = C3;
    hipStream_t side = nullptr;
    TCHK(hipStreamCreateWithFlags(&side, hipStreamNonBlocking));
    for (int r = 0; r < reps; ++r) {
        p.rev = r & 1;
        (void)hipMemcpyAsync(noise + ((r & 1) ? noise_bytes : 0), noise + ((r & 1) ? 0 : noise_bytes), noise_bytes, hipMemcpyDeviceToDevice, side);
        TCHK(hipMemsetAsync(p.y, 0xff, M * C2 * 2, nullptr));
        TCHK(hipMemsetAsync(p.z, 0xff, M * C3 * 2, nullptr));
        TCHK(opd_launch_btail(p, nullptr));
        TCHK(opd_launch_checksum(p.y, M * C2 * 2, sums + (size_t)(2 * r) * OPD_TAP_BLOCKS, nullptr));
        TCHK(opd_launch_checksum(p.z, M * C3 * 2, sums + (size_t)(2 * r + 1) * OPD_TAP_BLOCKS, nullptr));
    }
    TCHK(hipDeviceSynchronize());
    (void)hipStreamDestroy(side);
    std::vector<unsigned long long> h((size_t)reps * 2 * OPD_TAP_BLOCKS);
    TCHK(hipMemcpy(h.data(), sums, h.size() * 8, hipMemcpyDeviceToHost));
    int diff = 0;
    for (int r = 1; r < reps; ++r)
        if (memcmp(h.data() + (size_t)(2 * r) * OPD_TAP_BLOCKS, h.data(), 2 * OPD_TAP_BLOCKS * 8) != 0) ++diff;
    *n_diff = diff;
    return OPD_OK;
}

int opd_test_btail_sc(const uint16_t* x1, const uint16_t* w1, const float* b1, const uint16_t* w2, const float* b2sc, const uint16_t* xs,
                      const uint16_t* wsc, const uint16_t* w3, const float* b3, uint16_t* y, uint16_t* z, int B, int H, int W) {
    DevMem dm;
    const int C1 = 64, C2 = 256, C3 = 64;
    const size_t M = (size_t)B * H * W;
    std::vector<uint16_t> w2p((size_t)C2 * C1), w3p((size_t)C3 * C2);
    if (C1 == 256) {
        opd_permute_k32(w2, w2p.data(), C2, C1);
        opd_permute_k32(w3, w3p.data(), C3, C2);
    } else {
        w2p.assign(w2, w2 + (size_t)C2 * C1);
        w3p.assign(w3, w3 + (size_t)C3 * C2);
    }
    BtailParams p{}; p.dtype = g_test_dtype;
    p.x1 = dm.up(x1, M * C1);
    p.w1 = dm.up(w1, (size_t)C1 * 9 * C1);
    p.b1 = dm.up(b1, C1);
    p.w2p = dm.up(w2p.data(), w2p.size());
    p.b2 = dm.up(b2sc, C2);
    p.xs = dm.up(xs, M * 64);
    p.wsc = dm.up(wsc, (size_t)C2 * 64);
    p.y = dm.up<uint16_t>(nullptr, M * C2);
    p.w3p = dm.up(w3p.data(), w3p.size());
    p.b3 = dm.up(b3, C3);
    p.z = dm.up<uint16_t>(nullptr, M * C3);
    if (!p.x1 || !p.w1 || !p.b1 || !p.w2p || !p.b2 || !p.xs || !p.wsc || !p.y || !p.w3p || !p.b3 || !p.z) return tfail(OPD_ENOMEM, "test alloc failed");
    p.B = B; p.H = H; p.W = W; p.OH = H; p.OW = W; p.stride = 1; p.M = (int)M; p.C1 = C1; p.C3 = C3;
    TCHK(opd_launch_btail(p, nullptr));
    TCHK(hipDeviceSynchronize());
    TCHK(hipMemcpy(y, p.y, M * C2 * 2, hipMemcpyDeviceToHost));
    TCHK(hipMemcpy(z, p.z, M * C3 * 2, hipMemcpyDeviceToHost));
    return OPD_OK;
}

int opd_test_btail_chain(const uint16_t* x1, const uint16_t* xs, const uint16_t* const* w1, const float* const* b1, const uint16_t* const* w2,
                         const float* const* b2, const uint16_t* wsc, const uint16_t* const* w3, const float* const* b3, uint16_t* const* yb,
                         uint16_t* const* zb, uint16_t* const* yc, uint16_t* const* zc, int B, int H, int W, int fill) {
    DevMem dm;
    const size_t M = (size_t)B * H * W;
    const uint16_t* d_x1 = dm.up(x1, M * 64);
    const uint16_t* d_xs = dm.up(xs, M * 64);
    const uint16_t* d_wsc = dm.up(wsc, (size_t)256 * 64);
    const uint16_t *d_w1[3], *d_w2[3], *d_w3[3];
    const float *d_b1[3], *d_b2[3], *d_b3[3];
    for (int i = 0; i < 3; ++i) {
        const int c3 = i == 2 ? 128 : 64;
        d_w1[i] = dm.up(w1[i], (size_t)64 * 9 * 64); d_b1[i] = dm.up(b1[i], 64);
        d_w2[i] = dm.up(w2[i], (size_t)256 * 64); d_b2[i] = dm.up(b2[i], 256);
        d_w3[i] = dm.up(w3[i], (size_t)c3 * 256); d_b3[i] = dm.up(b3[i], c3);
        if (!d_w1[i] || !d_b1[i] || !d_w2[i] || !d_b2[i] || !d_w3[i] || !d_b3[i]) return tfail(OPD_ENOMEM, "test alloc failed");
    }
    uint16_t* ya = dm.up<uint16_t>(nullptr, M * 256);
    uint16_t* za = dm.up<uint16_t>(nullptr, M * 64);
    uint16_t* a1a = dm.up<uint16_t>(nullptr, M * 64);
    uint16_t* d_yb = dm.up<uint16_t>(nullptr, M * 256);
    uint16_t* d_zb = dm.up<uint16_t>(nullptr, M * 64);
    uint16_t* d_yc = dm.up<uint16_t>(nullptr, M * 256);
    uint16_t* d_zc = dm.up<uint16_t>(nullptr, M * 128);
    if (!d_x1 || !d_xs || !d_wsc || !ya || !za || !a1a || !d_yb || !d_zb || !d_yc || !d_zc) return tfail(OPD_ENOMEM, "test alloc failed");
    for (int route = 0; route < 2; ++route) {
        TCHK(hipMemset(ya, 0xEE, M * 256 * 2));
// ... 7 lines not shown
        BtailParams pa = base(0, d_x1, ya, za, 64);
        pa.xs = d_xs; pa.wsc = d_wsc;
        if (route) { pa.y = nullptr; pa.a1_out = a1a; }
        TCHK(opd_launch_btail(pa, nullptr));
        BtailParams pb = base(1, za, d_yb, d_zb, 64);
        if (route) { pb.rc = 1; pb.rc_a1 = a1a; pb.rc_xs = d_xs; pb.rc_w2 = d_w2[0]; pb.rc_wsc = d_wsc; pb.rc_b = d_b2[0]; }
        else pb.res = ya;
        TCHK(opd_launch_btail(pb, nullptr));
        BtailParams pc = base(2, d_zb, d_yc, d_zc, 128);
        pc.y_stride2 = route;
        pc.res = d_yb;
        TCHK(opd_launch_btail(pc, nullptr));
        TCHK(hipDeviceSynchronize());
        TCHK(hipMemcpy(yb[route], d_yb, M * 256 * 2, hipMemcpyDeviceToHost));
        TCHK(hipMemcpy(zb[route], d_zb, M * 64 * 2, hipMemcpyDeviceToHost));
        TCHK(hipMemcpy(yc[route], d_yc, M * 256 * 2, hipMemcpyDeviceToHost));
        TCHK(hipMemcpy(zc[route], d_zc, M * 128 * 2, hipMemcpyDeviceToHost));
    }
    return OPD_OK;
}

int opd_test_trace_btail(int B, int H, int W, int C1, int C3, int dbg, unsigned long long* trace_out, int max_wgs, int* wgs_out) {
    if (!opd_btail_supported(C1, C3)) return tfail(OPD_EINVAL, "btail: unsupported (C1, C3)");
    DevMem dm;
    const int C2 = 4 * C1;
    const size_t M = (size_t)B * H * W;
    const int wgs = (int)((M + 127) / 128);
    if (wgs > max_wgs) return tfail(OPD_EINVAL, "trace buffer too small");
    uint16_t* x1 = dm.up<uint16_t>(nullptr, M * C1);
    uint16_t* w1 = dm.up<uint16_t>(nullptr, (size_t)C1 * 9 * C1);
    uint16_t* w2 = dm.up<uint16_t>(nullptr, (size_t)C2 * C1);
    uint16_t* w3 = dm.up<uint16_t>(nullptr, (size_t)C3 * C2);
    float* bias = dm.up<float>(nullptr, C2);
    uint16_t* res = dm.up<uint16_t>(nullptr, M * C2);
    uint16_t* y = dm.up<uint16_t>(nullptr, M * C2);
    uint16_t* z = dm.up<uint16_t>(nullptr, M * C3);
    unsigned long long* tr = dm.up<unsigned long long>(nullptr, (size_t)wgs * 16);
    if (!x1 || !w1 || !w2 || !w3 || !bias || !res || !y || !z || !tr) return tfail(OPD_ENOMEM, "trace alloc failed");
    TCHK(hipMemset(x1, 0x2c, M * C1 * 2));
    TCHK(hipMemset(w1, 0x1c, (size_t)C1 * 9 * C1 * 2));
    TCHK(hipMemset(w2, 0x1c, (size_t)C2 * C1 * 2));
    TCHK(hipMemset(w3, 0x1c, (size_t)C3 * C2 * 2));
    TCHK(hipMemset(bias, 0, (size_t)C2 * 4));
    TCHK(hipMemset(res, 0x2c, M * C2 * 2));
    TCHK(hipMemset(tr, 0, (size_t)wgs * 128));
    BtailParams p{}; p.dtype = g_test_dtype;
    p.x1 = x1; p.w1 = w1; p.b1 = bias; p.w2p = w2; p.b2 = bias; p.res = res; p.y = y; p.w3p = w3; p.b3 = bias; p.z = z;
    p.B = B; p.H = H; p.W = W; p.OH = H; p.OW = W; p.stride = 1; p.M = (int)M; p.C1 = C1; p.C3 = C3; p.dbg = dbg;
    for (int i = 0; i < 2; ++i) TCHK(opd_launch_btail(p, nullptr));
    p.trace = tr;
    TCHK(opd_launch_btail(p, nullptr));
    TCHK(hipDeviceSynchronize());
    TCHK(hipMemcpy(trace_out, tr, (size_t)wgs * 128, hipMemcpyDeviceToHost));
    *wgs_out = wgs;
    return OPD_OK;
}

int opd_test_bench_btail(int B, int H, int W, int C1, int C3, int stride, int dbg, int iters, float* us_out) {
    if (!opd_btail_supported(C1, C3)) return tfail(OPD_EINVAL, "btail: unsupported (C1, C3)");
    DevMem dm;
    const int C2 = 4 * C1, OH = (H - 1) / stride + 1, OW = (W - 1) / stride + 1;
    const size_t M = (size_t)B * OH * OW;
    uint16_t* x1 = dm.up<uint16_t>(nullptr, (size_t)B * H * W * C1);
    uint16_t* w1 = dm.up<uint16_t>(nullptr, (size_t)C1 * 9 * C1);
    uint16_t* w2 = dm.up<uint16_t>(nullptr, (size_t)C2 * C1);
    uint16_t* w3 = dm.up<uint16_t>(nullptr, (size_t)(C3 ? C3 : 64) * C2);
    float* bias = dm.up<float>(nullptr, C2);
    uint16_t* res = dm.up<uint16_t>(nullptr, M * C2);
    uint16_t* a1 = dm.up<uint16_t>(nullptr, M * C1);
    uint16_t* y = dm.up<uint16_t>(nullptr, M * C2);
    uint16_t* z = dm.up<uint16_t>(nullptr, M * (C3 ? C3 : 64));
    float* zero = dm.up<float>(nullptr, 4096);
    if (!x1 || !w1 || !w2 || !w3 || !bias || !res || !a1 || !y || !z || !zero) return tfail(OPD_ENOMEM, "bench alloc failed");
    TCHK(hipMemset(x1, 0x2c, (size_t)B * H * W * C1 * 2));
    TCHK(hipMemset(w1, 0x1c, (size_t)C1 * 9 * C1 * 2));
    TCHK(hipMemset(w2, 0x1c, (size_t)C2 * C1 * 2));
    TCHK(hipMemset(w3, 0x1c, (size_t)(C3 ? C3 : 64) * C2 * 2));
    TCHK(hipMemset(bias, 0, (size_t)C2 * 4));
    TCHK(hipMemset(res, 0x2c, M * C2 * 2));
    TCHK(hipMemset(zero, 0, 4096 * 4));
    BtailParams p{}; p.dtype = g_test_dtype;
    p.x1 = x1; p.w1 = w1; p.b1 = bias; p.w2p = w2; p.b2 = bias; p.res = res; p.y = y; p.w3p = w3; p.b3 = bias; p.z = z;
    p.B = B; p.H = H; p.W = W; p.OH = OH; p.OW = OW; p.stride = stride; p.M = (int)M; p.C1 = C1; p.C3 = C3; p.dbg = dbg;
    ConvGemmParams c[3] = {};
    c[0].x = x1; c[0].w = w1; c[0].out = a1; c[0].B = B; c[0].H = H; c[0].W = W; c[0].Cin = C1; c[0].OH = OH; c[0].OW = OW; c[0].N = C1;
    c[0].KH = c[0].KW = 3; c[0].stride = stride; c[0].pad = 1; c[0].K = 9 * C1;
    c[1].x = a1; c[1].w = w2; c[1].res16 = res; c[1].out = y; c[1].B = B; c[1].H = OH; c[1].W = OW; c[1].Cin = C1; c[1].OH = OH; c[1].OW = OW;
    c[1].N = C2; c[1].KH = c[1].KW = 1; c[1].stride = 1; c[1].K = C1;
    c[2].x = y; c[2].w = w3; c[2].out = z; c[2].B = B; c[2].H = OH; c[2].W = OW; c[2].Cin = C2; c[2].OH = OH; c[2].OW = OW; c[2].N = C3 ? C3 : 64;
    c[2].KH = c[2].KW = 1; c[2].stride = 1; c[2].K = C2;
    for (auto& q : c) { q.bias = bias; q.zero16 = zero; q.M = (int)M; q.relu = 1; }
    hipEvent_t ev[2];
    TCHK(hipEventCreate(&ev[0])); TCHK(hipEventCreate(&ev[1]));
    for (int k = 0; k < 4; ++k) {
        if (k == 3 && !C3) { us_out[3] = 0.f; break; }
        if (k > 0 && dbg) { us_out[k] = 0.f; continue; }
        for (int i = -2; i < iters; ++i) {
            if (i == 0) TCHK(hipEventRecord(ev[0], nullptr));
            if (k == 0) TCHK(opd_launch_btail(p, nullptr));
            else TCHK(opd_launch_conv_gemm(c[k - 1], nullptr));
        }
        TCHK(hipEventRecord(ev[1], nullptr));
        TCHK(hipEventSynchronize(ev[1]));
        float ms = 0.f;
        TCHK(hipEventElapsedTime(&ms, ev[0], ev[1]));
        us_out[k] = ms * 1000.f / iters;
    }
    (void)hipEventDestroy(ev[0]); (void)hipEventDestroy(ev[1]);
    return OPD_OK;
}

int opd_test_bench_attention(const uint16_t* q, const uint16_t* k, const uint16_t* v, int B, int heads, int Lq, int Lk, int ldq, int ldkv,
                             float scale, int iters, float* us_out) {
    DevMem dm;
    AttnParams p{}; p.dtype = g_test_dtype;
    p.q = dm.up(q, (size_t)B * Lq * ldq);
    p.k = dm.up(k, (size_t)B * Lk * ldkv);
    p.v = dm.up(v, (size_t)B * Lk * ldkv);
    p.o = dm.up<uint16_t>(nullptr, (size_t)B * Lq * heads * 32);
    if (!p.q || !p.k || !p.v || !p.o) return tfail(OPD_ENOMEM, "bench alloc failed");
    p.B = B; p.heads = heads; p.Lq = Lq; p.Lk = Lk; p.ldq = ldq; p.ldk = p.ldv = ldkv; p.ldo = heads * 32; p.scale = scale;
    hipEvent_t a, b;
    TCHK(hipEventCreate(&a)); TCHK(hipEventCreate(&b));
    for (int i = 0; i < 3; ++i) TCHK(opd_launch_attention(p, nullptr));
    TCHK(hipEventRecord(a, nullptr));
    for (int i = 0; i < iters; ++i) TCHK(opd_launch_attention(p, nullptr));
    TCHK(hipEventRecord(b, nullptr));
    TCHK(hipEventSynchronize(b));
    float ms = 0.f;
    TCHK(hipEventElapsedTime(&ms, a, b));
    (void)hipEventDestroy(a); (void)hipEventDestroy(b);
    *us_out = ms * 1000.f / iters;
    return OPD_OK;
}

int opd_test_trace_attention(const uint16_t* q, const uint16_t* k, const uint16_t* v, int B, int heads, int Lq, int Lk, int ldq, int ldkv,
                             float scale, unsigned long long* trace_out, int max_wgs, int* wgs_out) {
    DevMem dm;
    AttnParams p{}; p.dtype = g_test_dtype;
    p.q = dm.up(q, (size_t)B * Lq * ldq);
    p.k = dm.up(k, (size_t)B * Lk * ldkv);
    p.v = dm.up(v, (size_t)B * Lk * ldkv);
    p.o = dm.up<uint16_t>(nullptr, (size_t)B * Lq * heads * 32);
    const int total = ((Lq + 63) / 64) * heads * B, grid = 8 * ((total + 7) / 8);
    unsigned long long* tr = dm.up<unsigned long long>(nullptr, (size_t)grid * 12);
    if (!p.q || !p.k || !p.v || !p.o || !tr) return tfail(OPD_ENOMEM, "trace alloc failed");
    TCHK(hipMemset(tr, 0, (size_t)grid * 96));
    p.B = B; p.heads = heads; p.Lq = Lq; p.Lk = Lk; p.ldq = ldq; p.ldk = p.ldv = ldkv; p.ldo = heads * 32; p.scale = scale;
    for (int i = 0; i < 2; ++i) TCHK(opd_launch_attention(p, nullptr));
    p.trace = tr;
    TCHK(opd_launch_attention(p, nullptr));
    TCHK(hipDeviceSynchronize());
    const int n = grid < max_wgs ? grid : max_wgs;
    TCHK(hipMemcpy(trace_out, tr, (size_t)n * 96, hipMemcpyDeviceToHost));
    *wgs_out = n;
    return OPD_OK;
}

int opd_test_attention(const uint16_t* q, const uint16_t* k, const uint16_t* v, uint16_t* o, int B, int heads, int Lq, int Lk,
                       float scale) {
    DevMem dm;
    const int D = heads * 32;
    AttnParams p{}; p.dtype = g_test_dtype;
    p.q = dm.up(q, (size_t)B * Lq * D);
    p.k = dm.up(k, (size_t)B * Lk * D);
    p.v = dm.up(v, (size_t)B * Lk * D);
// ... 145 lines not shown
    HeadParams p{};
    p.hs = dm.up(hs, (size_t)rows * 256);
    p.ln_gamma = ln_g ? dm.up(ln_g, 256) : nullptr;
    p.ln_beta = ln_b ? dm.up(ln_b, 256) : nullptr;
    p.wc = tr(wc, ncls, 256); p.bc = dm.up(bc, ncls);
    p.w1 = tr(w1, 256, 256); p.b1 = dm.up(b1, 256);
    p.w2 = tr(w2, 256, 256); p.b2 = dm.up(b2, 256);
    p.w3 = tr(w3, 4, 256); p.b3 = dm.up(b3, 4);
    p.logits = dm.up<float>(nullptr, (size_t)rows * ncls);
    p.boxes = dm.up<float>(nullptr, (size_t)rows * 4);
    if (!p.hs || !p.wc || !p.bc || !p.w1 || !p.b1 || !p.w2 || !p.b2 || !p.w3 || !p.b3 || !p.logits || !p.boxes) return tfail(OPD_ENOMEM, "test alloc failed");
    p.rows = rows; p.ncls = ncls;
    if (!heads_frags(dm, p, wc, w1, w2, ncls)) return tfail(OPD_ENOMEM, "test alloc failed");
    TCHK(opd_launch_heads(p, nullptr));
    TCHK(hipDeviceSynchronize());
    TCHK(hipMemcpy(logits, p.logits, (size_t)rows * ncls * 4, hipMemcpyDeviceToHost));
    TCHK(hipMemcpy(boxes, p.boxes, (size_t)rows * 4 * 4, hipMemcpyDeviceToHost));
    return OPD_OK;
}

int opd_test_postprocess(const float* logits, const float* boxes, const int32_t* orig_hw, int B, int Q, int ncls, float threshold,
                         opd_det* records, int32_t* counts) {
    DevMem dm;
    PostParams p{};
    p.logits = dm.up(logits, (size_t)B * Q * ncls);
    p.boxes = dm.up(boxes, (size_t)B * Q * 4);
    p.orig_hw = dm.up(orig_hw, (size_t)B * 2);
    opd_det* rec = dm.up<opd_det>(nullptr, (size_t)B * Q);
    p.counts = dm.up<int32_t>(nullptr, B);
    if (!p.logits || !p.boxes || !p.orig_hw || !rec || !p.counts) return tfail(OPD_ENOMEM, "test alloc failed");
    TCHK(hipMemset(rec, 0, (size_t)B * Q * sizeof(opd_det)));
    p.records = rec; p.B = B; p.Q = Q; p.ncls = ncls; p.threshold = threshold;
    TCHK(opd_launch_postprocess(p, nullptr));
    TCHK(hipDeviceSynchronize());
    TCHK(hipMemcpy(records, rec, (size_t)B * Q * sizeof(opd_det), hipMemcpyDeviceToHost));
    TCHK(hipMemcpy(counts, p.counts, (size_t)B * 4, hipMemcpyDeviceToHost));
    return OPD_OK;
}

int opd_test_roi_features(const float* enc, const int32_t* rois, int n, int h, int w, float* out) {
    DevMem dm;
    const float* d_enc = dm.up(enc, (size_t)h * w * 256);
    const int32_t* d_rois = dm.up(rois, (size_t)n * 4);
    float* d_out = dm.up<float>(nullptr, (size_t)n * 256);
    if (!d_enc || !d_rois || !d_out) return tfail(OPD_ENOMEM, "test alloc failed");
    TCHK(opd_launch_roi_features(d_enc, d_rois, d_out, n, h, w, nullptr));
    TCHK(hipDeviceSynchronize());
    TCHK(hipMemcpy(out, d_out, (size_t)n * 256 * 4, hipMemcpyDeviceToHost));
    return OPD_OK;
}

uint16_t opd_test_f32_to_f16(float f) { return opd::f32_to_f16(f); }
float opd_test_f16_to_f32(uint16_t h) { return opd::f16_to_f32(h); }
int opd_test_normalise_key(const char* in, char* out, int cap) {
    const std::string k = opd::normalise_key(in);
    if ((int)k.size() + 1 > cap) return OPD_EINVAL;
    memcpy(out, k.c_str(), k.size() + 1);
    return OPD_OK;
}
int opd_test_inspect_checkpoint(const char* path, int32_t* info8) {
    opd::StateDict sd;
    std::string err;
    int rc = opd::load_safetensors(path, &sd, &err);
    if (rc) return tfail(rc, err);
    opd::Arch a;
    rc = opd::infer_arch(sd, &a, &err);
    if (rc) return tfail(rc, err);
    for (int i = 0; i < 4; ++i) info8[i] = a.depths[i];
    info8[4] = a.enc_layers; info8[5] = a.dec_layers; info8[6] = a.queries; info8[7] = a.ncls;
    return OPD_OK;
}


int opd_test_resize_coeffs(int in_size, int out_size, int32_t* bounds, int32_t* coeffs, int coeffs_capacity) {
    std::vector<int32_t> b, k;
    int ksize = 0;
    opd_resize_coeffs(in_size, out_size, &b, &k, &ksize);
    if ((int)k.size() > coeffs_capacity) return fail(OPD_EINVAL, "coefficient buffer too small");
    memcpy(bounds, b.data(), b.size() * 4);
    memcpy(coeffs, k.data(), k.size() * 4);
    return ksize;
}
int opd_test_valid_prefix(int valid, int in, int out) { return valid_prefix(valid, in, out); }
int opd_test_trunk_plan(const int* depths, int max_batch, int flags, int B, int H, int W, int num_cus, int* steps_out, int max_steps, int* split_out) {
    if (!depths || !steps_out || !split_out || B < 1 || H < 1 || W < 1 || num_cus < 1) return tfail(OPD_EINVAL, "bad trunk_plan arguments");
    Arch a;
    std::vector<Block> blocks;
    auto conv = [](int cin, int cout, int k, int stride) {
        Conv c;
        c.Cin = cin; c.Cout = cout; c.KH = c.KW = k; c.stride = stride; c.pad = k / 2; c.K = k * k * cin;
        return c;
    };
    for (int s = 0, cin = 64; s < 4; ++s) {
        a.depths[s] = depths[s];
        if (depths[s] < 1) return tfail(OPD_EINVAL, "every stage needs a block");
        const int cout = a.hidden[s], mid = cout / 4;
        for (int l = 0; l < depths[s]; ++l) {
            const int stride = (l == 0 && s > 0) ? 2 : 1;
            Block b;
            b.has_sc = l == 0;
            if (b.has_sc) b.sc = conv(cin, cout, 1, stride);
            b.c0 = conv(cin, mid, 1, 1); b.c1 = conv(mid, mid, 3, stride); b.c2 = conv(mid, cout, 1, 1);
            blocks.push_back(b);
            cin = cout;
        }
    }
    if ((int)blocks.size() > max_steps) return tfail(OPD_EINVAL, "steps_out too small");
    opd_config cfg{};
    cfg.struct_size = sizeof(opd_config); cfg.max_batch = max_batch; cfg.max_height = H; cfg.max_width = W; cfg.flags = flags;
    const TrunkPlan plan = plan_trunk(a, blocks, cfg, Switches{}, B, down2(down2(H)), down2(down2(W)), num_cus, false, 0, true);
    for (size_t i = 0; i < plan.steps.size(); ++i) {
        const TrunkStep& t = plan.steps[i];
        const int row[7] = {t.path, t.sc, t.res, t.store, t.C3, t.rev, t.rev_b};
        memcpy(steps_out + 7 * i, row, sizeof(row));
    }
    *split_out = plan.split;
    return (int)blocks.size();
}
int opd_test_sine_pos_embed(int h, int w, int vh, int vw, int D, float* out) {
    if (!out || h < 1 || w < 1 || vh < 1 || vw < 1 || vh > h || vw > w || D < 2 || (D & 1)) return fail(OPD_EINVAL, "bad sine_pos_embed arguments");
    std::vector<float> pos;
    sine_pos_embed(h, w, vh, vw, D, &pos);
    memcpy(out, pos.data(), pos.size() * sizeof(float));
    return OPD_OK;
}
int opd_test_set_fuse_gemm_ln(opd_detr* m, int on) {
    if (!m) return fail(OPD_EINVAL, "null model handle");
    m->sw.fuse_gemm_ln = on ? 1 : 0;
    m->sw.small_m_gemm = on ? 1 : 0;
    m->sw.deep_fc2 = on ? 1 : 0;
    m->sw.fuse_dec0 = on ? 1 : 0;
    m->sw.fused_dec = on ? 1 : 0;
    if (fill_qc0(m) != OPD_OK) return OPD_EHIP;
    for (auto& g : m->graphs)
        if (g.exec) (void)hipGraphExecDestroy(g.exec);
    m->graphs.clear();
    return OPD_OK;
}
int opd_test_set_fuse_btail(opd_detr* m, int on) {
    if (!m) return fail(OPD_EINVAL, "null model handle");
    m->sw.fuse_btail = (on & 1) ? 1 : 0;
    m->sw.fuse_shortcut = (on & 2) ? 1 : 0;
    for (auto& g : m->graphs)
        if (g.exec) (void)hipGraphExecDestroy(g.exec);
    m->graphs.clear();
    return OPD_OK;
}
int opd_test_set_pos_shadow(opd_detr* m, int on) {
    if (!m) return fail(OPD_EINVAL, "null model handle");
    m->sw.pos_shadow = on ? 1 : 0;
    for (auto& g : m->graphs)
        if (g.exec) (void)hipGraphExecDestroy(g.exec);
    m->graphs.clear();
    return OPD_OK;
}
int opd_test_set_fuse_stem_pool(opd_detr* m, int on) {
    if (!m) return fail(OPD_EINVAL, "null model handle");
    m->sw.fuse_stem_pool = (on & 1) ? 1 : 0;
    m->sw.fuse_prep = (on & 2) ? 1 : 0;
    for (auto& g : m->graphs)
        if (g.exec) (void)hipGraphExecDestroy(g.exec);
    m->graphs.clear();
    return OPD_OK;
}

int opd_test_set_alloc_poison(int byte) {
    g_alloc_poison = byte < 0 ? -1 : (byte & 255);
    return OPD_OK;
}
int opd_test_check_redzones(opd_detr* m) {
    ApiScope api_scope;
    if (!m) return fail(OPD_EINVAL, "null model handle");
    HIPCHK(hipSetDevice(m->device));
    HIPCHK(hipDeviceSynchronize());
    std::vector<unsigned char> h(OPD_REDZONE);
    int bad = 0;
    std::string first;
    auto scan = [&](const std::vector<RedZoned>& v, const char* what) -> int {
        for (size_t i = 0; i < v.size(); ++i)
            for (int side = 0; side < 2; ++side) {
                const char* z = static_cast<const char*>(v[i].base) + (side ? OPD_REDZONE + v[i].bytes : 0);
                HIPCHK(hipMemcpy(h.data(), z, OPD_REDZONE, hipMemcpyDeviceToHost));
                size_t lo = OPD_REDZONE, hi = 0;
                for (size_t k = 0; k < OPD_REDZONE; ++k)
                    if (h[k] != (unsigned char)v[i].poison) { lo = std::min(lo, k); hi = k; }
                if (lo <= hi) {
                    if (!bad++) first = std::string(what) + " buffer #" + std::to_string(i) + " (" + std::to_string(v[i].bytes) + " bytes): " +
                                        (side ? "zone BEHIND it" : "zone IN FRONT of it") + " overwritten at zone offsets " + std::to_string(lo) + " .. " + std::to_string(hi);
                }
            }
        return OPD_OK;
    };
    RCCHK(scan(m->zoned, "handle"));
    if (m->weights) RCCHK(scan(m->weights->zoned, "weight-set"));
    if (bad) g_err = first;
    return bad;
}
// ... 251 lines not shown
```

Baseline: 3081.

## Add halo-tiled fused bottleneck tail kernel for stage-2 stride-1 blocks

After: 3111, median of 6. No clear change (+1.0%).

```diff
diff --git a/office_person_detection_vit_amd/_capi.py b/office_person_detection_vit_amd/_capi.py
--- a/office_person_detection_vit_amd/_capi.py
+++ b/office_person_detection_vit_amd/_capi.py
@@ -145,6 +145,8 @@
     "opd_test_resize_coeffs": (C.c_int, [C.c_int, C.c_int, C.c_void_p, C.c_void_p, C.c_int]),
     "opd_test_valid_prefix": (C.c_int, [C.c_int] * 3),
     "opd_test_trunk_plan": (C.c_int, [C.c_void_p] + [C.c_int] * 6 + [C.c_void_p, C.c_int, C.c_void_p]),
+    "opd_test_trunk_plan_halo": (C.c_int, [C.c_void_p] + [C.c_int] * 7 + [C.c_void_p, C.c_void_p, C.c_int, C.c_void_p]),
+    "opd_test_set_btail_halo": (C.c_int, [C.c_int]),
     "opd_test_sine_pos_embed": (C.c_int, [C.c_int] * 5 + [C.c_void_p]),
     "opd_test_conv_dual": (C.c_int, [C.c_void_p] * 6 + [C.c_int] * 13),
     "opd_test_btail_sc": (C.c_int, [C.c_void_p] * 11 + [C.c_int] * 3),
diff --git a/office_person_detection_vit_amd/csrc/build.py b/office_person_detection_vit_amd/csrc/build.py
--- a/office_person_detection_vit_amd/csrc/build.py
+++ b/office_person_detection_vit_amd/csrc/build.py
@@ -7,9 +7,9 @@
 
 HERE = os.path.dirname(os.path.abspath(__file__))
 PKG = os.path.dirname(HERE)
-SOURCES = ["kernels_gemm.hip", "kernels_w8.hip", "kernels_btail.hip", "kernels_btail3.hip", "kernels_rowln.hip", "kernels_attn.hip", "kernels_misc.hip", "kernels_dec.hip", "kernels_reid.hip", "kernels_osnet.hip", "opd_loader.cpp", "opd_host.cpp", "opd_model.cpp", "opd_comm.cpp", "opd_dispatch.cpp", "opd_reid.cpp", "opd_osnet.cpp", "opd_test_api.cpp", "opd_reid_test_api.cpp", "opd_osnet_test_api.cpp"]
+SOURCES = ["kernels_gemm.hip", "kernels_w8.hip", "kernels_btail.hip", "kernels_btail2.hip", "kernels_btail3.hip", "kernels_rowln.hip", "kernels_attn.hip", "kernels_misc.hip", "kernels_dec.hip", "kernels_reid.hip", "kernels_osnet.hip", "opd_loader.cpp", "opd_host.cpp", "opd_model.cpp", "opd_comm.cpp", "opd_dispatch.cpp", "opd_reid.cpp", "opd_osnet.cpp", "opd_test_api.cpp", "opd_reid_test_api.cpp", "opd_osnet_test_api.cpp"]
 TEST_ONLY = {"opd_test_api.cpp", "opd_reid_test_api.cpp", "opd_osnet_test_api.cpp"}
-ELEM_SOURCES = ["kernels_gemm.hip", "kernels_w8.hip", "kernels_btail.hip", "kernels_btail3.hip", "kernels_rowln.hip", "kernels_attn.hip", "kernels_misc.hip"]
+ELEM_SOURCES = ["kernels_gemm.hip", "kernels_w8.hip", "kernels_btail.hip", "kernels_btail2.hip", "kernels_btail3.hip", "kernels_rowln.hip", "kernels_attn.hip", "kernels_misc.hip"]
 HEADERS = ["opd_kernels.h", "opd_elem.h", "opd_loader.h", "opd_host.h", "opd_model.h", "opd_reid.h", "opd_osnet.h", os.path.join("..", "..", "include", "opd_detr.h")]
 COMMON_FLAGS = ["-O3", "-fPIC", "-std=c++17", "--offload-arch=gfx950", "-Wall", "-Wno-unused-function", "-fvisibility=hidden"]
 EXTRA_FLAGS = {"kernels_attn.hip": ["-mllvm", "-amdgpu-mfma-vgpr-form"]}
diff --git a/office_person_detection_vit_amd/csrc/kernels_btail.hip b/office_person_detection_vit_amd/csrc/kernels_btail.hip
--- a/office_person_detection_vit_amd/csrc/kernels_btail.hip
+++ b/office_person_detection_vit_amd/csrc/kernels_btail.hip
@@ -526,6 +526,7 @@
     p.fd_ow = opd_make_fastdiv((unsigned)p.OW);
     if ((size_t)p.B * p.H * p.W * p.C1 * 2 + (size_t)(p.W + 1) * p.C1 * 2 >= 0x7fffff00ull) return hipErrorInvalidValue;
     if ((size_t)p.M * p.C1 * 8 >= 0x7fffff00ull) return hipErrorInvalidValue;
+    if (p.halo) return OPD_SYM(opd_launch_btail_halo)(p, stream);
     if (p.C1 == 256) return OPD_SYM(opd_launch_btail256)(p, stream);
     if (p.y_stride2 && (p.stride != 1 || p.C3 == 0)) return hipErrorInvalidValue;
     if (!p.y && !p.a1_out) return hipErrorInvalidValue;
diff --git a/office_person_detection_vit_amd/csrc/kernels_btail2.hip b/office_person_detection_vit_amd/csrc/kernels_btail2.hip
--- /dev/null
+++ b/office_person_detection_vit_amd/csrc/kernels_btail2.hip
@@ -0,0 +1,395 @@
+#include <hip/hip_runtime.h>
+#include "opd_kernels.h"
+#include "opd_elem.h"
+
+typedef elem_t half8 __attribute__((ext_vector_type(8)));
+typedef float float4v __attribute__((ext_vector_type(4)));
+typedef unsigned int uint4v __attribute__((ext_vector_type(4)));
+
+namespace {
+
+constexpr int ROW_BYTES = 128;
+constexpr int TH = 8, TW = 32;
+[[maybe_unused]] constexpr int PH = TH + 2, PW = TW + 2;
+constexpr int PROWS = 352;
+[[maybe_unused]] constexpr int PIECES_PER_HALF = PROWS / 8;
+
+__device__ __forceinline__ int swz(int row, int chunk) { return row * ROW_BYTES + ((chunk ^ (row & 7)) << 4); }
+
+__device__ __forceinline__ int xcd_logical_block(int bid, int nblocks) {
+    const int q = nblocks >> 3, r = nblocks & 7;
+    const int x = bid & 7, k = bid >> 3;
+    return (x < r ? x * (q + 1) : r * (q + 1) + (x - r) * q) + k;
+}
+__device__ __forceinline__ int xcd_logical_block_rev(int bid, int nblocks) {
+    const int q = nblocks >> 3, r = nblocks & 7;
+    const int x = bid & 7, k = bid >> 3;
+    return (x < r ? x * (q + 1) + q - k : r * (q + 1) + (x - r) * q + q - 1 - k);
+}
+__device__ __forceinline__ int own_row(const int rho) { return (rho & ~31) | (((rho >> 2) & 3) << 3) | (((rho >> 4) & 1) << 2) | (rho & 3); }
+__device__ __forceinline__ int own_ch(const int nt, const int g) { return (nt >> 1) * 32 + g * 8 + (nt & 1) * 4; }
+
+__device__ __forceinline__ unsigned pack2h(float a, float b) {
+    typedef elem_t half2v __attribute__((ext_vector_type(2)));
+    half2v h;
+    h[0] = (elem_t)a;
+    h[1] = (elem_t)b;
+    unsigned u;
+    __builtin_memcpy(&u, &h, 4);
+    return u;
+}
+__device__ __forceinline__ void unpack2h(unsigned u, float& a, float& b) {
+    typedef elem_t half2v __attribute__((ext_vector_type(2)));
+    half2v h;
+    __builtin_memcpy(&h, &u, 4);
+    a = (float)h[0];
+    b = (float)h[1];
+}
+__device__ __forceinline__ half8 as_half8(unsigned a, unsigned b, unsigned c, unsigned d) {
+    uint4v u = {a, b, c, d};
+    half8 h;
+    __builtin_memcpy(&h, &u, 16);
+    return h;
+}
+template <int N_OUTSTANDING>
+__device__ __forceinline__ void wait_vmcnt() {
+    static_assert(N_OUTSTANDING >= 0 && N_OUTSTANDING <= 63, "vmcnt range");
+    asm volatile("s_waitcnt vmcnt(%0)" ::"n"(N_OUTSTANDING) : "memory");
+}
+__device__ __forceinline__ void compiler_fence() { asm volatile("" ::: "memory"); }
+__device__ __forceinline__ void lds_barrier() { asm volatile("s_waitcnt lgkmcnt(0)\n\ts_barrier" ::: "memory"); }
+
+template <int C1>
+struct HaloLayout {
+    static constexpr int KPC = C1 / 64;
+    static constexpr int PATCH_HALF = PROWS * ROW_BYTES;
+    static constexpr int RING = KPC * PATCH_HALF;
+    static constexpr int SLOT = C1 * ROW_BYTES;
+    static constexpr int BIAS = RING + 3 * SLOT;
+    static constexpr int LDS = BIAS + (C1 + 4 * C1 + C1) * 4;
+    static constexpr int CHUNK = 64 * C1 * 2 + C1 * ROW_BYTES;
+};
+
+template <int C1, int C3>
+__global__ __launch_bounds__(512, 1) void btail_halo_kernel(BtailParams p) {
+#if defined(__HIP_DEVICE_COMPILE__)
+    static_assert(C1 == 128 && (C3 == 0 || C3 == 128), "stage-2 tails");
+    using L = HaloLayout<C1>;
+    static_assert(L::LDS <= 160 * 1024 && 2 * L::CHUNK <= L::RING && 64 * C1 * 2 <= L::SLOT && C3 * ROW_BYTES <= L::SLOT, "LDS map");
+    extern __shared__ __attribute__((aligned(16))) unsigned char smem[];
+    constexpr int C2 = 4 * C1;
+    constexpr int NT1 = C1 / 16;
+    constexpr int KK1 = C1 / 32;
+    constexpr int NCH = C2 / 64;
+    constexpr int NT3 = C3 / 16;
+    constexpr int W1_PIECES = C1 / 64;
+    constexpr int W2_PIECES = 64 * C1 * 2 / (1024 * 8);
+    constexpr int W3_PIECES = C3 / 64;
+    constexpr int P_PIECES = L::KPC * PIECES_PER_HALF / 8;
+    static_assert(P_PIECES * 8 == L::KPC * PIECES_PER_HALF, "patch pieces split evenly over the waves");
+    constexpr int nk = 9 * L::KPC;
+    static_assert(nk % 3 == 0, "the last k-step sits in ring slot 2");
+
+    const int tid = threadIdx.x;
+    const int lane = tid & 63;
+    const int wave = __builtin_amdgcn_readfirstlane(tid >> 6);
+    const int g = lane >> 4, li = lane & 15;
+
+    const int tiles_w = (p.OW + TW - 1) / TW, tiles_h = (p.OH + TH - 1) / TH;
+    const int t = p.rev ? xcd_logical_block_rev(blockIdx.x, gridDim.x) : xcd_logical_block(blockIdx.x, gridDim.x);
+    const int tpf = tiles_w * tiles_h;
+    const int b = __builtin_amdgcn_readfirstlane(t / tpf);
+    const int tr = t - b * tpf;
+    const int th = __builtin_amdgcn_readfirstlane(tr / tiles_w);
+    const int oh0 = th * TH, ow0 = (tr - th * tiles_w) * TW;
+    const int oh = oh0 + wave;
+
+    const int lrow = lane >> 3;
+    const int lchunk = (lane & 7) ^ lrow;
+    const __amdgpu_buffer_rsrc_t rsrc_a = __builtin_amdgcn_make_buffer_rsrc(const_cast<f16_t*>(p.x1), 0, (unsigned)((size_t)p.B * p.H * p.W * C1 * 2), 0x00020000);
+    const __amdgpu_buffer_rsrc_t rsrc_w1 = __builtin_amdgcn_make_buffer_rsrc(const_cast<f16_t*>(p.w1), 0, (unsigned)(C1 * 9 * C1 * 2), 0x00020000);
+    const __amdgpu_buffer_rsrc_t rsrc_w2 = __builtin_amdgcn_make_buffer_rsrc(const_cast<f16_t*>(p.w2p), 0, (unsigned)(C2 * C1 * 2), 0x00020000);
+    const __amdgpu_buffer_rsrc_t rsrc_w3 = __builtin_amdgcn_make_buffer_rsrc(const_cast<f16_t*>(C3 ? p.w3p : p.w2p), 0, (unsigned)((C3 ? C3 : 1) * C2 * 2), 0x00020000);
+    unsigned woff1[W1_PIECES], woff2[W2_PIECES], woff3[W3_PIECES ? W3_PIECES : 1];
+#pragma unroll
+    for (int i = 0; i < W1_PIECES; ++i) woff1[i] = (unsigned)(own_row((wave * W1_PIECES + i) * 8 + lrow) * (9 * C1)) * 2u + (unsigned)lchunk * 16u;
+#pragma unroll
+    for (int i = 0; i < W2_PIECES; ++i) {
+        const int q = wave * W2_PIECES + i;
+        woff2[i] = (unsigned)(own_row((q & 7) * 8 + lrow) * C1 + (q >> 3) * 64) * 2u + (unsigned)lchunk * 16u;
+    }
+#pragma unroll
+    for (int i = 0; i < W3_PIECES; ++i) woff3[i] = (unsigned)(own_row((wave * W3_PIECES + i) * 8 + lrow) * C2) * 2u + (unsigned)lchunk * 16u;
+
+    auto issue_patch = [&]() {
+#pragma unroll
+        for (int i = 0; i < P_PIECES; ++i) {
+            const int q = wave * P_PIECES + i;
+            const int half = q / PIECES_PER_HALF, row = (q - half * PIECES_PER_HALF) * 8 + lrow;
+            const int pr = row / PW, pc = row - pr * PW;
+            const int ih = oh0 - 1 + pr, iw = ow0 - 1 + pc;
+            const bool ok = row < PH * PW && (unsigned)ih < (unsigned)p.H && (unsigned)iw < (unsigned)p.W;
+            const unsigned vo = ok ? (unsigned)(((b * p.H + ih) * p.W + iw) * C1 + half * 64) * 2u + (unsigned)lchunk * 16u : 0x80000000u;
+            __builtin_amdgcn_raw_ptr_buffer_load_lds(rsrc_a, (__attribute__((address_space(3))) void*)(smem + q * 1024), 16, vo, 0, 0, 0);
+        }
+    };
+    auto issue_w1 = [&](int ks) {
+        unsigned char* Ws = smem + L::RING + (ks % 3) * L::SLOT;
+#pragma unroll
+        for (int i = 0; i < W1_PIECES; ++i)
+            __builtin_amdgcn_raw_ptr_buffer_load_lds(rsrc_w1, (__attribute__((address_space(3))) void*)(Ws + (wave * W1_PIECES + i) * 1024), 16, woff1[i],
+                                                     ks * 128, 0, 0);
+    };
+    auto w2_base = [&](int c) -> unsigned char* { return c == 0 ? smem + L::RING : smem + ((c - 1) & 1) * L::CHUNK; };
+    auto w3_base = [&](int c) -> unsigned char* { return c == 0 ? smem + L::RING + L::SLOT : smem + ((c - 1) & 1) * L::CHUNK + 64 * C1 * 2; };
+    auto issue_w2 = [&](int c) {
+#pragma unroll
+        for (int i = 0; i < W2_PIECES; ++i)
+            __builtin_amdgcn_raw_ptr_buffer_load_lds(rsrc_w2, (__attribute__((address_space(3))) void*)(w2_base(c) + (wave * W2_PIECES + i) * 1024), 16,
+                                                     woff2[i], c * (64 * C1 * 2), 0, 0);
+    };
+    auto issue_w3 = [&](int c) {
+        if constexpr (C3 > 0) {
+#pragma unroll
+            for (int i = 0; i < W3_PIECES; ++i)
+                __builtin_amdgcn_raw_ptr_buffer_load_lds(rsrc_w3, (__attribute__((address_space(3))) void*)(w3_base(c) + (wave * W3_PIECES + i) * 1024), 16,
+                                                         woff3[i], c * 128, 0, 0);
+        }
+    };
+
+    bool pr_ok[2];
+    unsigned yoff[2], zoff[2];
+#pragma unroll
+    for (int mt = 0; mt < 2; ++mt) {
+        const int ow = ow0 + mt * 16 + li;
+        pr_ok[mt] = oh < p.OH && ow < p.OW;
+        const unsigned m = (unsigned)((b * p.OH + oh) * p.OW + ow);
+        yoff[mt] = pr_ok[mt] ? m * (unsigned)(C2 * 2) + (unsigned)g * 16u : 0x80000000u;
+        zoff[mt] = pr_ok[mt] ? m * (unsigned)(C3 * 2) + (unsigned)g * 16u : 0x80000000u;
+    }
+    const unsigned y_bytes = (unsigned)((size_t)p.M * C2 * 2);
+    const bool has_res = p.res != nullptr && !(p.dbg & 4);
+    const __amdgpu_buffer_rsrc_t rsrc_r = __builtin_amdgcn_make_buffer_rsrc(const_cast<f16_t*>(has_res ? p.res : p.x1), 0, has_res ? y_bytes : 0u, 0x00020000);
+    const __amdgpu_buffer_rsrc_t rsrc_y = __builtin_amdgcn_make_buffer_rsrc(p.y, 0, (p.dbg & 2) ? 0u : y_bytes, 0x00020000);
+    auto load_res = [&](int j, uint4v (&r)[4]) {
+#pragma unroll
+        for (int i = 0; i < 4; ++i)
+            r[i] = __builtin_amdgcn_raw_buffer_load_b128(rsrc_r, yoff[i & 1] + (unsigned)(j * 64 + (i >> 1) * 32) * 2u, 0, 0);
+    };
+    const float* const bias = reinterpret_cast<const float*>(smem + L::BIAS);
+
+    issue_patch();
+    issue_w1(0);
+    issue_w1(1);
+    compiler_fence();
+    for (int i = tid; i < C1 + C2 + C3; i += 512)
+        const_cast<float*>(bias)[i] = i < C1 ? p.b1[i] : i < C1 + C2 ? p.b2[i - C1] : p.b3[i - C1 - C2];
+    wait_vmcnt<0>();
+    lds_barrier();
+    float4v acc1[NT1][2];
+#pragma unroll
+    for (int nt = 0; nt < NT1; ++nt) {
+        const float4v bb = *reinterpret_cast<const float4v*>(bias + own_ch(nt, g));
+        acc1[nt][0] = bb;
+        acc1[nt][1] = bb;
+    }
+    const int group = wave >> 2;
+    if (group == 1) lds_barrier();
+    half8 xf[2][2], wf[2][NT1];
+    int tap_kh = 0, tap_kw = 0, tap_c = 0;
+    auto read_frags = [&](int ks) {
+        const unsigned char* Ps = smem + tap_c * L::PATCH_HALF;
+        const unsigned char* Ws = smem + L::RING + (ks % 3) * L::SLOT;
+#pragma unroll
+        for (int kk = 0; kk < 2; ++kk) {
+#pragma unroll
+            for (int mt = 0; mt < 2; ++mt) xf[kk][mt] = *reinterpret_cast<const half8*>(Ps + swz((wave + tap_kh) * PW + mt * 16 + li + tap_kw, kk * 4 + g));
+#pragma unroll
+            for (int nt = 0; nt < NT1; ++nt) wf[kk][nt] = *reinterpret_cast<const half8*>(Ws + swz(nt * 16 + li, kk * 4 + g));
+        }
+        if (++tap_c == L::KPC) {
+            tap_c = 0;
+            if (++tap_kw == 3) { tap_kw = 0; ++tap_kh; }
+        }
+    };
+    auto mfma_phase = [&]() {
+        __builtin_amdgcn_s_setprio(1);
+#pragma unroll
+        for (int kk = 0; kk < 2; ++kk)
+#pragma unroll
+            for (int nt = 0; nt < NT1; ++nt)
+#pragma unroll
+                for (int mt = 0; mt < 2; ++mt) acc1[nt][mt] = OPD_MFMA_16x16x32(wf[kk][nt], xf[kk][mt], acc1[nt][mt]);
+        __builtin_amdgcn_s_setprio(0);
+        lds_barrier();
+    };
+#pragma unroll 1
+    for (int ks = 0; ks + 2 < nk; ++ks) {
+        read_frags(ks);
+        compiler_fence();
+        issue_w1(ks + 2);
+        wait_vmcnt<W1_PIECES>();
+        lds_barrier();
+        mfma_phase();
+    }
+    read_frags(nk - 2);
+    compiler_fence();
+    issue_w2(0);
+    wait_vmcnt<W2_PIECES>();
+    lds_barrier();
+    mfma_phase();
+    read_frags(nk - 1);
+    compiler_fence();
+    issue_w3(0);
+    compiler_fence();
+    uint4v res[3][4];
+    load_res(0, res[0]);
+    load_res(1, res[1]);
+    compiler_fence();
+    lds_barrier();
+    mfma_phase();
+    if (group == 0) lds_barrier();
+    wait_vmcnt<0>();
+    lds_barrier();
+
+    half8 a1[2][KK1];
+#pragma unroll
+    for (int mt = 0; mt < 2; ++mt)
+#pragma unroll
+        for (int kk = 0; kk < KK1; ++kk) {
+            float4v u = acc1[2 * kk][mt], v = acc1[2 * kk + 1][mt];
+#pragma unroll
+            for (int r = 0; r < 4; ++r) {
+                u[r] = u[r] > 0.f ? u[r] : 0.f;
+                v[r] = v[r] > 0.f ? v[r] : 0.f;
+            }
+            a1[mt][kk] = as_half8(pack2h(u[0], u[1]), pack2h(u[2], u[3]), pack2h(v[0], v[1]), pack2h(v[2], v[3]));
+        }
+    float4v accz[NT3 ? NT3 : 1][2];
+    if constexpr (C3 > 0) {
+#pragma unroll
+        for (int nt = 0; nt < NT3; ++nt) {
+            const float4v bb = *reinterpret_cast<const float4v*>(bias + C1 + C2 + own_ch(nt, g));
+            accz[nt][0] = bb;
+            accz[nt][1] = bb;
+        }
+    }
+    if (p.dbg & 8) return;
+
+#pragma unroll
+    for (int j = 0; j < NCH; ++j) {
+        uint4v (&res_cur)[4] = res[j % 3];
+        if (j + 1 < NCH) {
+            issue_w2(j + 1);
+            issue_w3(j + 1);
+        }
+        compiler_fence();
+        if (j + 2 < NCH) load_res(j + 2, res[(j + 2) % 3]);
+        compiler_fence();
+        const unsigned char* W2s = w2_base(j);
+        float4v acc2[4][2];
+#pragma unroll
+        for (int nt = 0; nt < 4; ++nt) {
+            const float4v bb = *reinterpret_cast<const float4v*>(bias + C1 + j * 64 + own_ch(nt, g));
+            acc2[nt][0] = bb;
+            acc2[nt][1] = bb;
+        }
+#pragma unroll
+        for (int kk = 0; kk < KK1; ++kk) {
+            half8 w[4];
+#pragma unroll
+            for (int nt = 0; nt < 4; ++nt) w[nt] = *reinterpret_cast<const half8*>(W2s + (kk >> 1) * 8192 + swz(nt * 16 + li, (kk & 1) * 4 + g));
+#pragma unroll
+            for (int nt = 0; nt < 4; ++nt)
+#pragma unroll
+                for (int mt = 0; mt < 2; ++mt) acc2[nt][mt] = OPD_MFMA_16x16x32(w[nt], a1[mt][kk], acc2[nt][mt]);
+        }
+        half8 yf[2][2];
+        uint4v yo[2][2];
+#pragma unroll
+        for (int q = 0; q < 2; ++q)
+#pragma unroll
+            for (int mt = 0; mt < 2; ++mt) {
+                float4v v0 = acc2[2 * q][mt], v1 = acc2[2 * q + 1][mt];
+                if (has_res) {
+                    const uint4v r = res_cur[2 * q + mt];
+                    float a, c;
+                    unpack2h(r[0], a, c); v0[0] += a; v0[1] += c;
+                    unpack2h(r[1], a, c); v0[2] += a; v0[3] += c;
+                    unpack2h(r[2], a, c); v1[0] += a; v1[1] += c;
+                    unpack2h(r[3], a, c); v1[2] += a; v1[3] += c;
+                }
+#pragma unroll
+                for (int r = 0; r < 4; ++r) {
+                    v0[r] = v0[r] > 0.f ? v0[r] : 0.f;
+                    v1[r] = v1[r] > 0.f ? v1[r] : 0.f;
+                }
+                yo[q][mt] = uint4v{pack2h(v0[0], v0[1]), pack2h(v0[2], v0[3]), pack2h(v1[0], v1[1]), pack2h(v1[2], v1[3])};
+                yf[q][mt] = as_half8(yo[q][mt][0], yo[q][mt][1], yo[q][mt][2], yo[q][mt][3]);
+            }
+        if constexpr (C3 > 0) {
+            const unsigned char* W3s = w3_base(j);
+#pragma unroll
+            for (int kk = 0; kk < 2; ++kk) {
+#pragma unroll
+                for (int nt = 0; nt < NT3; ++nt) {
+                    const half8 w = *reinterpret_cast<const half8*>(W3s + swz(nt * 16 + li, kk * 4 + g));
+#pragma unroll
+                    for (int mt = 0; mt < 2; ++mt) accz[nt][mt] = OPD_MFMA_16x16x32(w, yf[kk][mt], accz[nt][mt]);
+                }
+            }
+        }
+        if (j + 1 < NCH) {
+            wait_vmcnt<0>();
+            lds_barrier();
+        }
+#pragma unroll
+        for (int q = 0; q < 2; ++q)
+#pragma unroll
+            for (int mt = 0; mt < 2; ++mt)
+                __builtin_amdgcn_raw_buffer_store_b128(yo[q][mt], rsrc_y, yoff[mt] + (unsigned)(j * 64 + q * 32) * 2u, 0, 0);
+    }
+
+    if constexpr (C3 > 0) {
+        const __amdgpu_buffer_rsrc_t rsrc_z = __builtin_amdgcn_make_buffer_rsrc(p.z, 0, (p.dbg & 2) ? 0u : (unsigned)((size_t)p.M * C3 * 2), 0x00020000);
+#pragma unroll
+        for (int q = 0; q < NT3 / 2; ++q)
+#pragma unroll
+            for (int mt = 0; mt < 2; ++mt) {
+                float4v v0 = accz[2 * q][mt], v1 = accz[2 * q + 1][mt];
+#pragma unroll
+                for (int r = 0; r < 4; ++r) {
+                    v0[r] = v0[r] > 0.f ? v0[r] : 0.f;
+                    v1[r] = v1[r] > 0.f ? v1[r] : 0.f;
+                }
+                __builtin_amdgcn_raw_buffer_store_b128(uint4v{pack2h(v0[0], v0[1]), pack2h(v0[2], v0[3]), pack2h(v1[0], v1[1]), pack2h(v1[2], v1[3])},
+                                                       rsrc_z, zoff[mt] + (unsigned)(q * 32) * 2u, 0, 0);
+            }
+    }
+#endif
+}
+
+template <int C1, int C3>
+hipError_t launch_halo_t(const BtailParams& p, hipStream_t stream) {
+    constexpr int LDS = HaloLayout<C1>::LDS;
+    const long long tiles = (long long)p.B * ((p.OH + TH - 1) / TH) * ((p.OW + TW - 1) / TW);
+    OPD_SET_MAX_LDS_ONCE((btail_halo_kernel<C1, C3>), LDS);
+    OPD_LAUNCH((btail_halo_kernel<C1, C3>), dim3((unsigned)tiles), dim3(512), LDS, stream, p);
+    static const char* const kname = opd_kernel_name("btail_halo_kernel<%d, %d>", C1, C3);
+    opd_last_kernel_name = kname;
+    return hipGetLastError();
+}
+
+}
+
+#ifndef OPD_ELEM_BF16
+bool opd_btail_halo_supported(const BtailParams& p) {
+    return p.C1 == 128 && (p.C3 == 0 || p.C3 == 128) && p.stride == 1 && p.OH == p.H && p.OW == p.W && !p.xs && !p.rc && !p.a1_out && !p.y_stride2 &&
+           !p.trace && p.y;
+}
+#endif
+
+hipError_t OPD_SYM(opd_launch_btail_halo)(const BtailParams& p, hipStream_t stream) {
+    if (!opd_btail_halo_supported(p)) return hipErrorInvalidValue;
+    return p.C3 ? launch_halo_t<128, 128>(p, stream) : launch_halo_t<128, 0>(p, stream);
+}
diff --git a/office_person_detection_vit_amd/csrc/opd_kernels.h b/office_person_detection_vit_amd/csrc/opd_kernels.h
--- a/office_person_detection_vit_amd/csrc/opd_kernels.h
+++ b/office_person_detection_vit_amd/csrc/opd_kernels.h
@@ -113,12 +113,14 @@
     const float* rc_b;
     int rc;
     int y_stride2;
+    int halo;
 };
 bool opd_btail_supported(int C1, int C3);
 hipError_t opd_launch_btail(const BtailParams& p, hipStream_t stream);
 void opd_permute_k32(const f16_t* w, f16_t* out, int rows, int K);
 bool opd_btail256_supported(int C1, int C3);
 hipError_t opd_launch_btail256(const BtailParams& p, hipStream_t stream);
+bool opd_btail_halo_supported(const BtailParams& p);
 
 struct GemmLnParams {
     const f16_t* x;
@@ -320,6 +322,7 @@
               hipStream_t stream)
 OPD_DECL_ELEM(opd_launch_btail, const BtailParams& p, hipStream_t stream)
 OPD_DECL_ELEM(opd_launch_btail256, const BtailParams& p, hipStream_t stream)
+OPD_DECL_ELEM(opd_launch_btail_halo, const BtailParams& p, hipStream_t stream)
 OPD_DECL_ELEM(opd_launch_gemm_ln, const GemmLnParams& p, hipStream_t stream)
 OPD_DECL_ELEM(opd_launch_enc_ffn, const EncFfnParams& p, hipStream_t stream)
 OPD_DECL_ELEM(opd_launch_gemm_k256, const GemmK256Params& p, hipStream_t stream)
diff --git a/office_person_detection_vit_amd/csrc/opd_model.cpp b/office_person_detection_vit_amd/csrc/opd_model.cpp
--- a/office_person_detection_vit_amd/csrc/opd_model.cpp
+++ b/office_person_detection_vit_amd/csrc/opd_model.cpp
@@ -693,6 +693,12 @@
                     prev.store = STORE_A1;
                     t.res = RES_REBUILD;
                 }
+            }
+            t.halo = 0;
+            if (tail && sw.tail_halo && C1 == 128 && b.c1.stride == 1 && t.sc == SC_NONE && t.res == RES_TRUNK && t.store == STORE_Y &&
+                (t.C3 == 0 || t.C3 == 128)) {
+                const long long tiles = (long long)cfg.max_batch * ((oh + 7) / 8) * ((ow + 31) / 32);
+                t.halo = 2 * tiles >= num_cus ? 1 : 0;
             }
             if (s == 2 && l == 0) { oh3 = oh; ow3 = ow; }
             ch = oh; cw = ow;
@@ -857,6 +863,7 @@
                     p.B = nb; p.H = ch; p.W = cw; p.OH = oh; p.OW = ow; p.stride = b.c1.stride; p.M = nb * oh * ow; p.C1 = C1; p.C3 = C3;
                     p.rev = b0 ? t.rev_b : t.rev;
                     p.dbg = m->sw.dbg_btail;
+                    p.halo = t.halo;
                     RCCHK(timed_begin(m, CLS_CONV, 2.0 * p.M * ((double)C1 * 9 * C1 + 4.0 * C1 * C1 + 4.0 * C1 * C3 + (t.sc == SC_TAIL ? 64.0 * 256 : 0.0))));
                     HIPCHK(opd_launch_btail(p, m->stream));
                     RCCHK(timed_end(m));
@@ -1355,6 +1362,7 @@
     env("OPD_TAIL_REV", &sw.tail_rev);
     env("OPD_TAIL3", &sw.tail3);
     env("OPD_TAIL_RC", &sw.tail_rc);
+    env("OPD_TAIL_HALO", &sw.tail_halo);
     sw.tail_rc = sw.tail_rc != 0;
     env("OPD_WPREFETCH", &sw.wprefetch);
     env("OPD_W8", &sw.w8);
diff --git a/office_person_detection_vit_amd/csrc/opd_model.h b/office_person_detection_vit_amd/csrc/opd_model.h
--- a/office_person_detection_vit_amd/csrc/opd_model.h
+++ b/office_person_detection_vit_amd/csrc/opd_model.h
@@ -113,6 +113,7 @@
     int tail3 = 1;
     int tail3_split = 1;
     int tail_rc = 1;
+    int tail_halo = 1;
     int y_stride2 = 1;
     int wprefetch = 3;
     int w8 = -1;
@@ -135,6 +136,7 @@
     int path, sc, res, store;
     int C3;
     int rev, rev_b;
+    int halo;
 };
 struct TrunkPlan {
     std::vector<TrunkStep> steps;
diff --git a/office_person_detection_vit_amd/csrc/opd_test_api.cpp b/office_person_detection_vit_amd/csrc/opd_test_api.cpp
--- a/office_person_detection_vit_amd/csrc/opd_test_api.cpp
+++ b/office_person_detection_vit_amd/csrc/opd_test_api.cpp
@@ -37,6 +37,8 @@
 
 static int g_conv_flags = 0, g_gemm_ln_kloop = 0, g_test_dtype = 0;
 int opd_test_set_elem_bf16(int on) { g_test_dtype = on ? OPD_DT_BF16 : OPD_DT_F16; return OPD_OK; }
+static int g_test_btail_halo = 0, g_test_btail_rev = 0;
+int opd_test_set_btail_halo(int bits) { g_test_btail_halo = bits & 1; g_test_btail_rev = (bits >> 1) & 1; return OPD_OK; }
 int opd_test_set_conv_flags(int flags) { g_conv_flags = flags; return OPD_OK; }
 int opd_test_set_gemm_ln_kloop(int on) { g_gemm_ln_kloop = on ? 1 : 0; return OPD_OK; }
 static void apply_conv_flags(ConvGemmParams& p, int flags) {
@@ -421,6 +423,8 @@
     if (!p.x1 || !p.w1 || !p.b1 || !p.w2p || !p.b2 || !p.y || (res && !p.res) || (C3 && (!p.w3p || !p.b3 || !p.z)))
         return tfail(OPD_ENOMEM, "test alloc failed");
     p.B = B; p.H = H; p.W = W; p.OH = OH; p.OW = OW; p.stride = stride; p.M = (int)M; p.C1 = C1; p.C3 = C3;
+    p.halo = g_test_btail_halo;
+    p.rev = g_test_btail_rev;
     TCHK(opd_launch_btail(p, nullptr));
     TCHK(hipDeviceSynchronize());
     TCHK(hipMemcpy(y, p.y, M * C2 * 2, hipMemcpyDeviceToHost));
@@ -451,6 +455,7 @@
     unsigned long long* sums = dm.up<unsigned long long>(nullptr, (size_t)reps * 2 * OPD_TAP_BLOCKS);
     if (!p.x1 || !p.w1 || !p.b1 || !p.w2p || !p.b2 || !p.res || !p.y || !p.w3p || !p.b3 || !p.z || !noise || !sums) return tfail(OPD_ENOMEM, "test alloc failed");
     p.B = B; p.H = H; p.W = W; p.OH = H; p.OW = W; p.stride = 1; p.M = (int)M; p.C1 = C1; p.C3 = C3;
+    p.halo = g_test_btail_halo;
     hipStream_t side = nullptr;
     TCHK(hipStreamCreateWithFlags(&side, hipStreamNonBlocking));
     for (int r = 0; r < reps; ++r) {
@@ -624,6 +629,7 @@
     BtailParams p{}; p.dtype = g_test_dtype;
     p.x1 = x1; p.w1 = w1; p.b1 = bias; p.w2p = w2; p.b2 = bias; p.res = res; p.y = y; p.w3p = w3; p.b3 = bias; p.z = z;
     p.B = B; p.H = H; p.W = W; p.OH = OH; p.OW = OW; p.stride = stride; p.M = (int)M; p.C1 = C1; p.C3 = C3; p.dbg = dbg;
+    p.halo = g_test_btail_halo;
     ConvGemmParams c[3] = {};
     c[0].x = x1; c[0].w = w1; c[0].out = a1; c[0].B = B; c[0].H = H; c[0].W = W; c[0].Cin = C1; c[0].OH = OH; c[0].OW = OW; c[0].N = C1;
     c[0].KH = c[0].KW = 3; c[0].stride = stride; c[0].pad = 1; c[0].K = 9 * C1;
@@ -935,7 +941,20 @@
     return ksize;
 }
 int opd_test_valid_prefix(int valid, int in, int out) { return valid_prefix(valid, in, out); }
+static int trunk_plan_impl(const int* depths, int max_batch, int flags, int B, int H, int W, int num_cus, const Switches& sw, int* steps_out,
+                           int* halo_out, int max_steps, int* split_out);
 int opd_test_trunk_plan(const int* depths, int max_batch, int flags, int B, int H, int W, int num_cus, int* steps_out, int max_steps, int* split_out) {
+    return trunk_plan_impl(depths, max_batch, flags, B, H, W, num_cus, Switches{}, steps_out, nullptr, max_steps, split_out);
+}
+int opd_test_trunk_plan_halo(const int* depths, int max_batch, int flags, int B, int H, int W, int num_cus, int tail_halo, int* steps_out, int* halo_out,
+                             int max_steps, int* split_out) {
+    if (!halo_out) return tfail(OPD_EINVAL, "bad trunk_plan arguments");
+    Switches sw;
+    sw.tail_halo = tail_halo;
+    return trunk_plan_impl(depths, max_batch, flags, B, H, W, num_cus, sw, steps_out, halo_out, max_steps, split_out);
+}
+static int trunk_plan_impl(const int* depths, int max_batch, int flags, int B, int H, int W, int num_cus, const Switches& sw, int* steps_out,
+                           int* halo_out, int max_steps, int* split_out) {
     if (!depths || !steps_out || !split_out || B < 1 || H < 1 || W < 1 || num_cus < 1) return tfail(OPD_EINVAL, "bad trunk_plan arguments");
     Arch a;
     std::vector<Block> blocks;
@@ -961,11 +980,12 @@
     if ((int)blocks.size() > max_steps) return tfail(OPD_EINVAL, "steps_out too small");
     opd_config cfg{};
     cfg.struct_size = sizeof(opd_config); cfg.max_batch = max_batch; cfg.max_height = H; cfg.max_width = W; cfg.flags = flags;
-    const TrunkPlan plan = plan_trunk(a, blocks, cfg, Switches{}, B, down2(down2(H)), down2(down2(W)), num_cus, false, 0, true);
+    const TrunkPlan plan = plan_trunk(a, blocks, cfg, sw, B, down2(down2(H)), down2(down2(W)), num_cus, false, 0, true);
     for (size_t i = 0; i < plan.steps.size(); ++i) {
         const TrunkStep& t = plan.steps[i];
         const int row[7] = {t.path, t.sc, t.res, t.store, t.C3, t.rev, t.rev_b};
         memcpy(steps_out + 7 * i, row, sizeof(row));
+        if (halo_out) halo_out[i] = t.halo;
     }
     *split_out = plan.split;
     return (int)blocks.size();
```
